# serycjon/WOFT

Hardware: AMD Instinct MI355X
Metric: tracked frames/sec at 1080p, 12 RAFT iters; flow EPE vs reference (higher is better)
Workload: dtype bf16x3 (split-bf16 MFMA operands emulating fp32, fp32 accumulate)

## Files before the change

### include/woft_hip.h

```cpp
#ifndef WOFT_HIP_H
#define WOFT_HIP_H

#include <stdint.h>

#ifdef __cplusplus
extern "C" {
#endif

#define WOFT_OK 0
#define WOFT_EINVAL (-1)
#define WOFT_ELAUNCH (-2)

int woft_abi_version(void);
int woft_sizeof(int which);
int woft_set_tuning(int key, int value);

enum woft_epilogue {
    WOFT_EPI_LINEAR = 0,
    WOFT_EPI_RELU = 1,
    WOFT_EPI_SIGMOID = 2,
    WOFT_EPI_TANH = 3,
    WOFT_EPI_RELU_RES_RELU = 4,
    WOFT_EPI_GRU_ZR = 5,
    WOFT_EPI_GRU_Q = 6,
// ... 63 lines not shown
int woft_flow_head_update(const float* in, int32_t cs, int32_t h, int32_t w, int32_t cin_pad, const float* wgt,
                          const float* bias, float* delta, int64_t ld_delta, float* coords1, float* flow4,
                          float* flow_cat, int32_t ld_cat, void* stream);
int woft_flow_head_gather(const float* part, int32_t n_planes, int32_t ld, int32_t h, int32_t w, const float* bias2,
                          float* delta, int64_t ld_delta, float* coords1, float* flow4, float* flow_cat, int32_t ld_cat,
                          void* stream);
int woft_split_bf16_lines(const float* x, int64_t n, void* out, void* stream);
int woft_corr_gemm_bf16(const void* a, const void* b, int64_t m, int64_t n, int64_t rows_a, int64_t rows_b, int32_t k,
                        float alpha, void* out, int64_t ldo, int32_t terms, int32_t out_bf16, void* stream);

int woft_inorm_finalize(const float* stat_sum, const float* stat_sq, int32_t n_part, int32_t ld,
                        int32_t channels, int32_t channels_pad, int64_t count, float eps,
                        float* mean, float* rstd, void* ws, void* stream);
int64_t woft_inorm_ws_bytes(void);
int woft_inorm_apply(const float* x, const float* mean, const float* rstd, const float* res,
                     const float* res_mean, const float* res_rstd, int32_t res_mode,
                     float* out, int64_t n_pix, int32_t channels, int32_t mode, void* stream);

int woft_preprocess_bgr_u8(const uint8_t* img, int32_t h, int32_t w, float* out,
                           int32_t hp, int32_t wp, int32_t pad_top, int32_t pad_left, void* stream);

int woft_avgpool2_nhwc(const float* in, int32_t h, int32_t w, int32_t c, float* out, void* stream);

int woft_feature_pyramid(const float* in, int32_t h, int32_t w, int32_t c, int32_t levels, float* const* pooled,
                         void* const* split, int32_t terms, void* stream);

typedef struct woft_lookup_params {
    const void* vol[4];
    int32_t ht[4], wt[4];
    int64_t plane[4];
    int32_t levels, radius;
    const float* coords;
    int64_t n_pix;
    float* out;
    int32_t ldo;
    int32_t vol_bf16;
    int32_t ablate;
} woft_lookup_params;
int woft_corr_lookup(const woft_lookup_params* p, void* stream);
typedef struct woft_lookup_otf_params {
    const void* f1;
    const void* f2[4];
    int32_t h[4], w[4];
    int32_t levels, radius, terms;
    int32_t hf, wf, k;
    float alpha;
    const float* coords;
    float* out;
    const int32_t* need;
    int32_t ldo;
    int32_t ablate;
    const float* fh_part;
    const float* fh_bias;
    float* fh_delta;
    float* fh_flow4;
    float* fh_flow_cat;
    int32_t fh_planes, fh_ld, fh_ld_delta, fh_ld_cat;
    int32_t roi_y0, roi_x0, roi_h, roi_w;
    int32_t smp_y0, smp_x0, smp_h, smp_w;
} woft_lookup_otf_params;
int woft_corr_lookup_otf(const woft_lookup_otf_params* p, void* stream);
int woft_tile_rows(const float* in, int32_t h, int32_t w, int32_t c, float* out, void* stream);

int woft_coords_update(float* coords1, const float* delta, int32_t ld_delta, int32_t wf, int64_t n_pix,
                       float* flow4, float* flow_cat, int32_t ld_cat, void* stream);
int woft_coords_init(float* coords1, int32_t hf, int32_t wf, float* flow4, float* flow_cat,
                     int32_t ld_cat, void* stream);
int woft_coords_init_flow(float* coords1, const float* flow_init, int32_t hf, int32_t wf, float* flow4, float* flow_cat,
                          int32_t ld_cat, void* stream);
int woft_forward_interpolate(const float* flow, int32_t hf, int32_t wf, float* out, void* stream);

int woft_colsum(const float* f, int64_t n_pix, int32_t c, double* ws, int32_t n_part, double* total, void* stream);
int woft_wh_conv0(const float* lookup, int32_t ld_lookup, const float* mean, int64_t n_pix, int32_t nwin,
                  const float* wt, const float* bias, float* out, const int32_t* index, void* stream);
int woft_wh_pack(const float* lookup, int32_t ld_lookup, const float* f1, int32_t c, const double* f2_total,
                 float alpha, int64_t n_pix, int32_t nwin, float* mean, float* x8, void* stream);
int woft_wh_reduce(const float* act, int32_t c, int32_t nwin2, const float* w, float bias,
                   int64_t n_pix, float* out, void* stream);
int woft_warp_features(const float* f, int32_t h, int32_t w, int32_t c, int32_t cs, const float* coords, int64_t n_pix,
                       float* out, int32_t ld_out, void* stream);
int woft_wh_needed(const float* pts, const int32_t* count, int32_t n_max, int32_t top, int32_t left, int32_t hf, int32_t wf,
                   const int32_t* index, int32_t n_win, int32_t* bitmap, int32_t* dyn_index, int32_t* n_needed, void* stream);

int woft_convex_upsample(const float* coords1, const float* wlow, const float* mask, int32_t ld_mask,
                         int32_t hf, int32_t wf, int32_t crop_top, int32_t crop_left, int32_t h, int32_t w,
                         float* flow_up, float* dst, float* wout, int32_t do_sigmoid, void* stream);
int woft_convex_weights_at(const float* pts, const int32_t* count, int32_t n_max, const float* wlow, const float* mask,
                           int32_t ld_mask, int32_t hf, int32_t wf, int32_t crop_top, int32_t crop_left,
                           int32_t do_sigmoid, float* wsel, void* stream);
int woft_flow_to_tc(const float* flow, const float* weights, int32_t h, int32_t w, float* dst, float* wout,
                    int32_t do_sigmoid, void* stream);
int woft_upflow8(const float* coords1, const float* wlow, int32_t hf, int32_t wf,
                 int32_t crop_top, int32_t crop_left, int32_t h, int32_t w,
                 float* flow_up, float* dst, float* wout, int32_t do_sigmoid, void* stream);

int woft_warp_perspective_u8(const uint8_t* img, int32_t h, int32_t w, int32_t c, const double* hinv,
                             uint8_t* out, uint8_t* valid, int32_t nearest, void* stream);

int woft_warp_perspective_window_u8(const uint8_t* img, int32_t h, int32_t w, int32_t c, const double* hinv, int32_t y0,
                                    int32_t x0, int32_t hw, int32_t ww, uint8_t* out, uint8_t* valid, int32_t nearest,
                                    void* stream);
int woft_crop_u8(const uint8_t* img, int32_t h, int32_t w, int32_t c, int32_t y0, int32_t x0, int32_t hw, int32_t ww,
                 uint8_t* out, void* stream);
int64_t woft_mask_bbox_ws_bytes(void);
int woft_mask_bbox(const uint8_t* mask, int32_t h, int32_t w, const double* hinv, uint8_t* warped, void* ws, int32_t* bbox,
                   void* stream);

int woft_resize_linear_u8(const uint8_t* img, int32_t h, int32_t w, int32_t c, uint8_t* out, int32_t ho, int32_t wo,
                          float scale_y, float scale_x, void* stream);

int64_t woft_tc_select_ws_bytes(int64_t n);
int woft_tc_select(const float* dst, const float* w, const uint8_t* tmask, const uint8_t* pwmask, int32_t gh,
                   int32_t gw, int32_t mh, int32_t mw, int32_t check_dst, const float* sobol_u, int32_t n_draw,
                   void* ws, float* pa, float* pb, float* wout, int32_t cap, int32_t* count, void* stream);
int woft_tc_flags(const float* dst, const uint8_t* tmask, const uint8_t* pwmask, int32_t gh, int32_t gw, int32_t mh,
                  int32_t mw, int32_t check_dst, uint8_t* flags, void* stream);
int woft_tc_select_vis(const float* dst, const float* w, const uint8_t* tmask, const uint8_t* pwmask, int32_t gh,
                       int32_t gw, int32_t mh, int32_t mw, int32_t check_dst, const float* sobol_u, int32_t n_draw,
                       const float* vis, int32_t vis_mode, float vis_thr, void* ws, float* pa, float* pb, float* wout,
                       int32_t cap, int32_t* count, void* stream);
int woft_tc_flags_vis(const float* dst, const uint8_t* tmask, const uint8_t* pwmask, int32_t gh, int32_t gw, int32_t mh,
                      int32_t mw, int32_t check_dst, const float* vis, int32_t vis_mode, float vis_thr, uint8_t* flags,
                      void* stream);

#define WOFT_HFIT_SINGLE_MAX 2048
int64_t woft_hfit_ws_bytes(void);
int woft_hfit(const float* pa, const float* pb, const float* w, int32_t n_max, const int32_t* count,
              int32_t reweight, float huber_k, int32_t n_irls, void* ws, float* Hout, int32_t* status, void* stream);
#define WOFT_HFIT_BATCH_MAX 65535
int woft_hfit_batched(const float* pa, const float* pb, const float* w, int32_t batch, int32_t n_max,
                      const int32_t* counts, int32_t reweight, float huber_k, int32_t n_irls, float* Hout,
                      int32_t* status, void* stream);
int woft_hfit_batched_bwd(const float* pa, const float* pb, const float* w, int32_t batch, int32_t n_max,
                          const int32_t* counts, const float* gH, float* gpa, float* gpb, float* gw, int32_t* status,
                          void* stream);
int woft_hfit_step(const float* pa, const float* pb, const float* w, int32_t n, const float* rew, int32_t first,
                   void* ws, float* res, float* Hout, int32_t* status, void* stream);
int woft_inlier_frac(const float* pa, const float* pb, int32_t n_max, const int32_t* count, const float* H,
                     float thr, float* frac, void* stream);

int64_t woft_ransac_ws_bytes(int32_t n_max, int32_t max_iters);
int woft_ransac(const float* pa, const float* pb, int32_t n_max, const int32_t* count, int32_t max_iters, double thr,
                double conf, uint64_t seed, int32_t refine, void* ws, float* Hout, int32_t* status, int32_t* info,
                uint8_t* inlier_mask, void* stream);

int64_t woft_trs_ws_bytes(int32_t n_max, int32_t max_iters);
int woft_trs(const float* pa, const float* pb, int32_t n_max, const int32_t* count, int32_t max_iters, double thr,
             double conf, uint64_t seed, int32_t refine, void* ws, float* Hout, int32_t* status, int32_t* info,
             uint8_t* inlier_mask, void* stream);

#ifdef __cplusplus
}
#endif
#endif
```

### woft_amd/_lib.py

```python
import ctypes as C
import os
from pathlib import Path

import torch

LIB_PATH = Path(os.environ.get("WOFT_HIP_LIB") or Path(__file__).resolve().parent / "lib" / "libwoft_hip.so")

EPI_LINEAR, EPI_RELU, EPI_SIGMOID, EPI_TANH, EPI_RELU_RES_RELU, EPI_GRU_ZR, EPI_GRU_Q, EPI_CTX, EPI_WH_MEAN, EPI_FLOWHEAD = range(10)

vp, i32, i64, f32 = C.c_void_p, C.c_int32, C.c_int64, C.c_float


class ConvParams(C.Structure):
    _fields_ = [
        ("in0", vp), ("in1", vp), ("cs0", i32), ("cs1", i32), ("c_split", i32),
        ("n_img", i32), ("h", i32), ("w", i32), ("ho", i32), ("wo", i32),
        ("taps_y", i32), ("taps_x", i32), ("stride", i32), ("pad_y", i32), ("pad_x", i32),
        ("cin_pad", i32), ("flat", i32), ("wgt", vp), ("wgt_hi", vp), ("wgt_lo", vp), ("precision", i32),
        ("bias", vp), ("alpha", f32),
        ("cout", i32), ("cout_pad", i32), ("out", vp), ("ldo", i64), ("co_off", i32),
        ("out_w", i32), ("out_pitch", i32), ("epi", i32), ("split", i32),
        ("e0", vp), ("e1", vp), ("lde0", i32), ("lde1", i32), ("out1", vp), ("ldo1", i32),
        ("stat_sum", vp), ("stat_sq", vp), ("tile_m", i32), ("tile_n", i32), ("halo", i32),
        ("in_norm", i32), ("in_mean", vp), ("in_rstd", vp), ("bias_map", vp), ("ld_bias_map", i32),
        ("out_index", vp),
        ("wh0_lookup", vp), ("wh0_ld", i32), ("wh0_mean", vp), ("wh0_w", vp), ("wh0_bias", vp), ("wh0_index", vp),
        ("wgt_frag", vp), ("wgt_mx", vp),
        ("roi_y0", i32), ("roi_x0", i32), ("roi_h", i32), ("roi_w", i32),
    ]


class LookupParams(C.Structure):
    _fields_ = [
        ("vol", vp * 4), ("ht", i32 * 4), ("wt", i32 * 4), ("plane", i64 * 4),
        ("levels", i32), ("radius", i32), ("coords", vp), ("n_pix", i64), ("out", vp), ("ldo", i32),
        ("vol_bf16", i32), ("ablate", i32),
    ]


class LookupOtfParams(C.Structure):
    _fields_ = [
        ("f1", vp), ("f2", vp * 4), ("h", i32 * 4), ("w", i32 * 4),
        ("levels", i32), ("radius", i32), ("terms", i32), ("hf", i32), ("wf", i32), ("k", i32),
        ("alpha", f32), ("coords", vp), ("out", vp), ("need", vp), ("ldo", i32), ("ablate", i32),
        ("fh_part", vp), ("fh_bias", vp), ("fh_delta", vp), ("fh_flow4", vp), ("fh_flow_cat", vp),
        ("fh_planes", i32), ("fh_ld", i32), ("fh_ld_delta", i32), ("fh_ld_cat", i32),
        ("roi_y0", i32), ("roi_x0", i32), ("roi_h", i32), ("roi_w", i32),
        ("smp_y0", i32), ("smp_x0", i32), ("smp_h", i32), ("smp_w", i32),
    ]


_SIGS = {
    "woft_abi_version": (i32, []),
    "woft_sizeof": (i32, [i32]),
    "woft_set_tuning": (i32, [i32, i32]),
    "woft_conv2d": (i32, [C.POINTER(ConvParams), vp]),
    "woft_conv2d_pair": (i32, [C.POINTER(ConvParams), C.POINTER(ConvParams), vp]),
    "woft_upload_u8": (i32, [vp, vp, vp, i64, i32, vp]),
    "woft_split_bf16": (i32, [vp, i64, vp, vp, vp]),
    "woft_split_bf16_lines": (i32, [vp, i64, vp, vp]),
    "woft_flow_to_tc": (i32, [vp, vp, i32, i32, vp, vp, i32, vp]),
    "woft_corr_lookup_otf": (i32, [C.POINTER(LookupOtfParams), vp]),
    "woft_conv3x3_narrow": (i32, [vp, i32, i32, i32, i32, i32, vp, vp, i32, vp, i64, i32, vp]),
    "woft_flow_head_update": (i32, [vp, i32, i32, i32, i32, vp, vp, vp, i64, vp, vp, vp, i32, vp]),
    "woft_flow_head_gather": (i32, [vp, i32, i32, i32, i32, vp, vp, i64, vp, vp, vp, i32, vp]),
    "woft_corr_gemm_bf16": (i32, [vp, vp, i64, i64, i64, i64, i32, f32, vp, i64, i32, i32, vp]),
    "woft_inorm_finalize": (i32, [vp, vp, i32, i32, i32, i32, i64, f32, vp, vp, vp, vp]),
    "woft_inorm_ws_bytes": (i64, []),
    "woft_inorm_apply": (i32, [vp, vp, vp, vp, vp, vp, i32, vp, i64, i32, i32, vp]),
    "woft_preprocess_bgr_u8": (i32, [vp, i32, i32, vp, i32, i32, i32, i32, vp]),
    "woft_avgpool2_nhwc": (i32, [vp, i32, i32, i32, vp, vp]),
    "woft_feature_pyramid": (i32, [vp, i32, i32, i32, i32, vp, vp, i32, vp]),
    "woft_corr_lookup": (i32, [C.POINTER(LookupParams), vp]),
    "woft_tile_rows": (i32, [vp, i32, i32, i32, vp, vp]),
    "woft_coords_update": (i32, [vp, vp, i32, i32, i64, vp, vp, i32, vp]),
    "woft_coords_init": (i32, [vp, i32, i32, vp, vp, i32, vp]),
    "woft_coords_init_flow": (i32, [vp, vp, i32, i32, vp, vp, i32, vp]),
    "woft_forward_interpolate": (i32, [vp, i32, i32, vp, vp]),
    "woft_colsum": (i32, [vp, i64, i32, vp, i32, vp, vp]),
    "woft_wh_pack": (i32, [vp, i32, vp, i32, vp, f32, i64, i32, vp, vp, vp]),
    "woft_wh_conv0": (i32, [vp, i32, vp, i64, i32, vp, vp, vp, vp, vp]),
    "woft_wh_reduce": (i32, [vp, i32, i32, vp, f32, i64, vp, vp]),
    "woft_warp_features": (i32, [vp, i32, i32, i32, i32, vp, i64, vp, i32, vp]),
    "woft_wh_needed": (i32, [vp, vp, i32, i32, i32, i32, i32, vp, i32, vp, vp, vp, vp]),
    "woft_convex_upsample": (i32, [vp, vp, vp, i32, i32, i32, i32, i32, i32, i32, vp, vp, vp, i32, vp]),
    "woft_convex_weights_at": (i32, [vp, vp, i32, vp, vp, i32, i32, i32, i32, i32, i32, vp, vp]),
    "woft_upflow8": (i32, [vp, vp, i32, i32, i32, i32, i32, i32, vp, vp, vp, i32, vp]),
    "woft_warp_perspective_u8": (i32, [vp, i32, i32, i32, C.POINTER(C.c_double), vp, vp, i32, vp]),
    "woft_resize_linear_u8": (i32, [vp, i32, i32, i32, vp, i32, i32, f32, f32, vp]),
    "woft_warp_perspective_window_u8": (i32, [vp, i32, i32, i32, C.POINTER(C.c_double), i32, i32, i32, i32, vp, vp, i32, vp]),
    "woft_crop_u8": (i32, [vp, i32, i32, i32, i32, i32, i32, i32, vp, vp]),
    "woft_mask_bbox_ws_bytes": (i64, []),
    "woft_mask_bbox": (i32, [vp, i32, i32, C.POINTER(C.c_double), vp, vp, vp, vp]),
    "woft_tc_select_ws_bytes": (i64, [i64]),
    "woft_tc_select": (i32, [vp, vp, vp, vp, i32, i32, i32, i32, i32, vp, i32, vp, vp, vp, vp, i32, vp, vp]),
    "woft_tc_flags": (i32, [vp, vp, vp, i32, i32, i32, i32, i32, vp, vp]),
    "woft_tc_select_vis": (i32, [vp, vp, vp, vp, i32, i32, i32, i32, i32, vp, i32, vp, i32, f32, vp, vp, vp, vp, i32, vp, vp]),
    "woft_tc_flags_vis": (i32, [vp, vp, vp, i32, i32, i32, i32, i32, vp, i32, f32, vp, vp]),
    "woft_hfit_ws_bytes": (i64, []),
    "woft_hfit": (i32, [vp, vp, vp, i32, vp, i32, f32, i32, vp, vp, vp, vp]),
    "woft_hfit_batched": (i32, [vp, vp, vp, i32, i32, vp, i32, f32, i32, vp, vp, vp]),
    "woft_hfit_batched_bwd": (i32, [vp, vp, vp, i32, i32, vp, vp, vp, vp, vp, vp, vp]),
    "woft_hfit_step": (i32, [vp, vp, vp, i32, vp, i32, vp, vp, vp, vp, vp]),
    "woft_inlier_frac": (i32, [vp, vp, i32, vp, vp, f32, vp, vp]),
    "woft_ransac_ws_bytes": (i64, [i32, i32]),
    "woft_ransac": (i32, [vp, vp, i32, vp, i32, C.c_double, C.c_double, C.c_uint64, i32, vp, vp, vp, vp, vp, vp]),
    "woft_trs_ws_bytes": (i64, [i32, i32]),
    "woft_trs": (i32, [vp, vp, i32, vp, i32, C.c_double, C.c_double, C.c_uint64, i32, vp, vp, vp, vp, vp, vp]),
}

EXPORTS = tuple(_SIGS)
_lib = None


class WoftHipError(RuntimeError):
    pass


def load():
    global _lib
    if _lib is not None:
        return _lib
    if not LIB_PATH.exists():
        raise WoftHipError(f"{LIB_PATH} is missing: build it with `python -m woft_amd.build` "
                           "(hipcc --offload-arch=gfx950); woft_amd has no CPU fallback")
    lib = C.CDLL(str(LIB_PATH))
    for name, (res, args) in _SIGS.items():
        fn = getattr(lib, name)
        fn.restype, fn.argtypes = res, args
    if lib.woft_sizeof(0) != C.sizeof(ConvParams) or lib.woft_sizeof(1) != C.sizeof(LookupParams) \
            or lib.woft_sizeof(2) != C.sizeof(LookupOtfParams):
        raise WoftHipError("ctypes mirror of woft_conv_params / woft_lookup_params is out of sync with the library")
    _lib = lib
    return lib


def check(rc, what):
    if rc != 0:
        raise WoftHipError(f"{what} failed with code {rc}")


def ptr(t):
    return None if t is None else t.data_ptr()


_RAW_STREAM = getattr(torch._C, "_cuda_getCurrentRawStream", None) if os.environ.get("WOFT_RAW_STREAM", "1") != "0" else None
_CUR_DEV = torch.cuda.current_device


def stream_ptr():
    if _RAW_STREAM is None:
        return torch.cuda.current_stream().cuda_stream
    return _RAW_STREAM(_CUR_DEV())
```

### woft_amd/csrc/hfit.hip

```cpp
#include "common.h"
#include <algorithm>

namespace {

constexpr int HT = 1024;
constexpr int NG = 45;

__device__ __forceinline__ double wave_sum(double v) {
#pragma unroll
    for (int o = 32; o > 0; o >>= 1) v += __shfl_xor(v, o);
    return v;
}

template <int CNT>
__device__ void block_sum(double (&vals)[CNT], double* red , double* out ) {
    const int lane = threadIdx.x & 63, wave = threadIdx.x >> 6;
#pragma unroll
    for (int i = 0; i < CNT; ++i) {
        const double s = wave_sum(vals[i]);
        if (lane == 0) red[wave * CNT + i] = s;
    }
    __syncthreads();
    if ((int)threadIdx.x < CNT) {
        double s = 0.0;
        for (int wv = 0; wv < HT / 64; ++wv) s += red[wv * CNT + threadIdx.x];
        out[threadIdx.x] = s;
    }
    __syncthreads();
}

__device__ __forceinline__ void build_rows(float x1, float y1, float x2, float y2, float wv, float (&rx)[9],
                                           float (&ry)[9]) {
    rx[0] = 0.f; rx[1] = 0.f; rx[2] = 0.f; rx[3] = -x1; rx[4] = -y1; rx[5] = -1.f; rx[6] = y2 * x1; rx[7] = y2 * y1;
    rx[8] = -y2;
    ry[0] = x1; ry[1] = y1; ry[2] = 1.f; ry[3] = 0.f; ry[4] = 0.f; ry[5] = 0.f; ry[6] = -x2 * x1; ry[7] = -x2 * y1;
    ry[8] = x2;
#pragma unroll
    for (int k = 0; k < 9; ++k) {
        rx[k] *= wv;
        ry[k] *= wv;
    }
}

__device__ __forceinline__ float reweight_fn(float r, int mode, float k) {
    const float a = fabsf(r);
    if (mode == 2 && a < k) return 1.f;
    return 1.f / (a + 1e-8f);
}

__device__ __forceinline__ void hfit_one(const float* __restrict__ pa, const float* __restrict__ pb,
                                         const float* __restrict__ w, int n, int reweight, float huber_k, int n_solves,
                                         float* __restrict__ Hout, int* __restrict__ status) {
    __shared__ double red[(HT / 64) * 81];
    __shared__ double tot[NG];
    __shared__ double gram[81];
    __shared__ float sol_s[8];
    __shared__ int fail_s;
    if (n < 4) {
        if (threadIdx.x == 0) {
            status[0] = 1;
            for (int i = 0; i < 9; ++i) Hout[i] = nanf("");
        }
        return;
    }
    if (threadIdx.x == 0) fail_s = 0;

    double s4[4] = {0.0, 0.0, 0.0, 0.0};
    for (int i = threadIdx.x; i < n; i += HT) {
        s4[0] += (double)pa[2 * i];
        s4[1] += (double)pa[2 * i + 1];
        s4[2] += (double)pb[2 * i];
        s4[3] += (double)pb[2 * i + 1];
    }
    block_sum<4>(s4, red, tot);
    const float m1x = (float)(tot[0] / n), m1y = (float)(tot[1] / n);
    const float m2x = (float)(tot[2] / n), m2y = (float)(tot[3] / n);
    __syncthreads();
    double d2[2] = {0.0, 0.0};
    for (int i = threadIdx.x; i < n; i += HT) {
        const float ax = pa[2 * i] - m1x, ay = pa[2 * i + 1] - m1y;
        const float bx = pb[2 * i] - m2x, by = pb[2 * i + 1] - m2y;
        d2[0] += (double)sqrtf(ax * ax + ay * ay);
        d2[1] += (double)sqrtf(bx * bx + by * by);
    }
    block_sum<2>(d2, red, tot);
    const float s1 = sqrtf(2.0f) / ((float)(tot[0] / n) + 1e-8f);
    const float s2 = sqrtf(2.0f) / ((float)(tot[1] / n) + 1e-8f);
    const float t1x = -s1 * m1x, t1y = -s1 * m1y, t2x = -s2 * m2x, t2y = -s2 * m2y;
    __syncthreads();

    typedef double f64x4 __attribute__((ext_vector_type(4)));
    const int lane = threadIdx.x & 63, wave = threadIdx.x >> 6;
    const int ec = lane & 15, ek = lane >> 4;
    for (int it = 0; it < n_solves; ++it) {
        float sol[8];
#pragma unroll
        for (int k = 0; k < 8; ++k) sol[k] = (it > 0) ? sol_s[k] : 0.f;
        f64x4 g4 = {0.0, 0.0, 0.0, 0.0};
        for (int base = wave * 2; base < n; base += (HT / 64) * 2) {
            const int i = base + (ek >> 1);
            double val = 0.0;
            if (i < n && ec < 9) {
                const float x1 = s1 * pa[2 * i] + t1x, y1 = s1 * pa[2 * i + 1] + t1y;
                const float x2 = s2 * pb[2 * i] + t2x, y2 = s2 * pb[2 * i + 1] + t2y;
                const float wv = (w != nullptr) ? w[i] : 1.f;
                float rx[9], ry[9];
                build_rows(x1, y1, x2, y2, wv, rx, ry);
                float q = 1.f;
                if (it > 0 && reweight != 0) {
                    float resx = -rx[8], resy = -ry[8];
#pragma unroll
                    for (int k = 0; k < 8; ++k) {
                        resx += rx[k] * sol[k];
                        resy += ry[k] * sol[k];
                    }
                    q = sqrtf(reweight_fn((ek & 1) ? resy : resx, reweight, huber_k));
                }
                float e = 0.f;
#pragma unroll
                for (int k = 0; k < 9; ++k)
                    if (k == ec) e = (ek & 1) ? ry[k] : rx[k];
                val = (double)(e * q);
            }
            g4 = __builtin_amdgcn_mfma_f64_16x16x4f64(val, val, g4, 0, 0, 0);
        }
#pragma unroll
        for (int r = 0; r < 4; ++r) {
            const int row = ek + 4 * r;
            if (row < 9 && ec < 9) red[wave * 81 + row * 9 + ec] = g4[r];
        }
        __syncthreads();
        if (threadIdx.x < 81) {
            double sacc = 0.0;
            for (int wv = 0; wv < HT / 64; ++wv) sacc += red[wv * 81 + threadIdx.x];
            gram[threadIdx.x] = sacc;
        }
        __syncthreads();
        if (threadIdx.x == 0) {
            double L[8][8], rhs[8];
            double G[9][9];
            for (int a = 0; a < 9; ++a)
                for (int b = 0; b < 9; ++b) G[a][b] = gram[a * 9 + b];
            bool ok = true;
            for (int i = 0; i < 8 && ok; ++i) {
                for (int j = 0; j <= i; ++j) {
                    double s = G[i][j];
                    for (int k = 0; k < j; ++k) s -= L[i][k] * L[j][k];
                    if (i == j) {
                        if (!(s > 0.0)) { ok = false; break; }
                        L[i][i] = sqrt(s);
                    } else {
                        L[i][j] = s / L[j][j];
                    }
                }
            }
            if (ok) {
                for (int i = 0; i < 8; ++i) {
                    double s = G[i][8];
                    for (int k = 0; k < i; ++k) s -= L[i][k] * rhs[k];
                    rhs[i] = s / L[i][i];
                }
                for (int i = 7; i >= 0; --i) {
                    double s = rhs[i];
                    for (int k = i + 1; k < 8; ++k) s -= L[k][i] * rhs[k];
                    rhs[i] = s / L[i][i];
                }
                for (int i = 0; i < 8; ++i) sol_s[i] = (float)rhs[i];
            } else {
                fail_s = 1;
            }
        }
        __syncthreads();
        if (fail_s) break;
    }

    if (threadIdx.x == 0) {
        if (fail_s) {
            status[0] = 2;
            for (int i = 0; i < 9; ++i) Hout[i] = nanf("");
            return;
        }
        const double hn[9] = {sol_s[0], sol_s[1], sol_s[2], sol_s[3], sol_s[4], sol_s[5], sol_s[6], sol_s[7], 1.0};
        const double T1[9] = {s1, 0, t1x, 0, s1, t1y, 0, 0, 1};
        const double i2 = 1.0 / (double)s2;
        const double T2i[9] = {i2, 0, -(double)t2x * i2, 0, i2, -(double)t2y * i2, 0, 0, 1};
        double tmp[9], hh[9];
        for (int r = 0; r < 3; ++r)
            for (int c = 0; c < 3; ++c) {
                double s = 0;
                for (int k = 0; k < 3; ++k) s += hn[r * 3 + k] * T1[k * 3 + c];
                tmp[r * 3 + c] = s;
            }
        for (int r = 0; r < 3; ++r)
            for (int c = 0; c < 3; ++c) {
                double s = 0;
                for (int k = 0; k < 3; ++k) s += T2i[r * 3 + k] * tmp[k * 3 + c];
                hh[r * 3 + c] = s;
            }
        const double den = hh[8] + 1e-8;
        for (int i = 0; i < 9; ++i) Hout[i] = (float)(hh[i] / den);
        status[0] = 0;
    }
}

__global__ __launch_bounds__(HT) void hfit_kernel(const float* __restrict__ pa, const float* __restrict__ pb,
                                                  const float* __restrict__ w, int n_max,
                                                  const int* __restrict__ count, int reweight, float huber_k,
                                                  int n_solves, float* __restrict__ Hout, int* __restrict__ status) {
    int n = n_max;
    if (count != nullptr) n = min(count[0], n_max);
    hfit_one(pa, pb, w, n, reweight, huber_k, n_solves, Hout, status);
}

__global__ __launch_bounds__(HT) void hfit_batched_kernel(const float* __restrict__ pa, const float* __restrict__ pb,
                                                          const float* __restrict__ w, int n_max,
                                                          const int* __restrict__ counts, int reweight, float huber_k,
                                                          int n_solves, float* __restrict__ Hout,
                                                          int* __restrict__ status) {
    const int b = blockIdx.x;
    const int64_t off = (int64_t)b * n_max;
    int n = n_max;
    if (counts != nullptr) n = min(counts[b], n_max);
    hfit_one(pa + 2 * off, pb + 2 * off, (w != nullptr) ? w + off : nullptr, n, reweight, huber_k, n_solves, Hout + 9 * b,
             status + b);
}


__device__ __forceinline__ bool chol8_factor(const double* gram, double (&L)[36]) {
    bool ok = true;
#pragma unroll
    for (int i = 0; i < 8; ++i) {
#pragma unroll
        for (int j = 0; j <= i; ++j) {
            double s = gram[i * 9 + j];
#pragma unroll
            for (int k = 0; k < j; ++k) s -= L[i * (i + 1) / 2 + k] * L[j * (j + 1) / 2 + k];
            if (i == j) {
                ok = ok && (s > 0.0);
                L[i * (i + 1) / 2 + i] = sqrt(s);
            } else {
                L[i * (i + 1) / 2 + j] = s / L[j * (j + 1) / 2 + j];
            }
        }
    }
    return ok;
}

__device__ __forceinline__ void chol8_solve_f64(const double (&L)[36], double (&rhs)[8]) {
#pragma unroll
    for (int i = 0; i < 8; ++i) {
        double s = rhs[i];
#pragma unroll
        for (int k = 0; k < i; ++k) s -= L[i * (i + 1) / 2 + k] * rhs[k];
        rhs[i] = s / L[i * (i + 1) / 2 + i];
    }
#pragma unroll
    for (int i = 7; i >= 0; --i) {
        double s = rhs[i];
#pragma unroll
        for (int k = i + 1; k < 8; ++k) s -= L[k * (k + 1) / 2 + i] * rhs[k];
        rhs[i] = s / L[i * (i + 1) / 2 + i];
    }
}

__device__ __forceinline__ void bwd_zero_rows(float* __restrict__ gpa, float* __restrict__ gpb, float* __restrict__ gw, int from,
                                              int n_max) {
    for (int i = from + (int)threadIdx.x; i < n_max; i += HT) {
        if (gpa != nullptr) ((float2*)gpa)[i] = make_float2(0.f, 0.f);
        if (gpb != nullptr) ((float2*)gpb)[i] = make_float2(0.f, 0.f);
        if (gw != nullptr) gw[i] = 0.f;
    }
}

__device__ __forceinline__ void hfit_bwd_one(const float* __restrict__ pa, const float* __restrict__ pb,
                                             const float* __restrict__ w, int n, int n_max, const float* __restrict__ gout,
                                             float* __restrict__ gpa, float* __restrict__ gpb, float* __restrict__ gw,
                                             int* __restrict__ status) {
    __shared__ double red[(HT / 64) * 81];
    __shared__ double tot[NG];
    __shared__ double gram[81];
    __shared__ double bw[24];
    __shared__ int fail_s;
    if (n < 4) {
        bwd_zero_rows(gpa, gpb, gw, 0, n_max);
        if (threadIdx.x == 0 && status != nullptr) status[0] = 1;
        return;
    }

    double s4[4] = {0.0, 0.0, 0.0, 0.0};
    for (int i = threadIdx.x; i < n; i += HT) {
        s4[0] += (double)pa[2 * i];
        s4[1] += (double)pa[2 * i + 1];
        s4[2] += (double)pb[2 * i];
        s4[3] += (double)pb[2 * i + 1];
    }
    block_sum<4>(s4, red, tot);
    const float m1x = (float)(tot[0] / n), m1y = (float)(tot[1] / n);
    const float m2x = (float)(tot[2] / n), m2y = (float)(tot[3] / n);
    __syncthreads();
    double d2[2] = {0.0, 0.0};
    for (int i = threadIdx.x; i < n; i += HT) {
        const float ax = pa[2 * i] - m1x, ay = pa[2 * i + 1] - m1y;
        const float bx = pb[2 * i] - m2x, by = pb[2 * i + 1] - m2y;
        d2[0] += (double)sqrtf(ax * ax + ay * ay);
        d2[1] += (double)sqrtf(bx * bx + by * by);
    }
    block_sum<2>(d2, red, tot);
    const float den1 = (float)(tot[0] / n) + 1e-8f, den2 = (float)(tot[1] / n) + 1e-8f;
    const float s1 = sqrtf(2.0f) / den1;
    const float s2 = sqrtf(2.0f) / den2;
    const float t1x = -s1 * m1x, t1y = -s1 * m1y, t2x = -s2 * m2x, t2y = -s2 * m2y;
    __syncthreads();

    typedef double f64x4 __attribute__((ext_vector_type(4)));
    const int lane = threadIdx.x & 63, wave = threadIdx.x >> 6;
    const int ec = lane & 15, ek = lane >> 4;
    {
        f64x4 g4 = {0.0, 0.0, 0.0, 0.0};
        for (int base = wave * 2; base < n; base += (HT / 64) * 2) {
            const int i = base + (ek >> 1);
            double val = 0.0;
            if (i < n && ec < 9) {
                const float x1 = s1 * pa[2 * i] + t1x, y1 = s1 * pa[2 * i + 1] + t1y;
                const float x2 = s2 * pb[2 * i] + t2x, y2 = s2 * pb[2 * i + 1] + t2y;
                const float wv = (w != nullptr) ? w[i] : 1.f;
                float rx[9], ry[9];
                build_rows(x1, y1, x2, y2, wv, rx, ry);
                float e = 0.f;
#pragma unroll
                for (int k = 0; k < 9; ++k)
                    if (k == ec) e = (ek & 1) ? ry[k] : rx[k];
                val = (double)e;
            }
            g4 = __builtin_amdgcn_mfma_f64_16x16x4f64(val, val, g4, 0, 0, 0);
        }
#pragma unroll
        for (int r = 0; r < 4; ++r) {
            const int row = ek + 4 * r;
            if (row < 9 && ec < 9) red[wave * 81 + row * 9 + ec] = g4[r];
        }
        __syncthreads();
        if (threadIdx.x < 81) {
            double sacc = 0.0;
            for (int wv = 0; wv < HT / 64; ++wv) sacc += red[wv * 81 + threadIdx.x];
            gram[threadIdx.x] = sacc;
        }
// ... 98 lines not shown
                for (int k = 0; k < 8; ++k) {
                    aUx += (double)ax[k] * bw[8 + k];
                    aXx += (double)ax[k] * bw[k];
                    aUy += (double)ay[k] * bw[8 + k];
                    aXy += (double)ay[k] * bw[k];
                }
                gw[i] = (float)((vX * (double)ax[8] - (rX * aUx + vX * aXx)) + (vY * (double)ay[8] - (rY * aUy + vY * aXy)));
            }
            if (want_pts) {
                const double W = (double)wv, X1 = x1, Y1 = y1, X2 = x2, Y2 = y2;
                const double gAx3 = -(rX * bw[11] + vX * bw[3]), gAx4 = -(rX * bw[12] + vX * bw[4]);
                const double gAx6 = -(rX * bw[14] + vX * bw[6]), gAx7 = -(rX * bw[15] + vX * bw[7]);
                const double gAy0 = -(rY * bw[8] + vY * bw[0]), gAy1 = -(rY * bw[9] + vY * bw[1]);
                const double gAy6 = -(rY * bw[14] + vY * bw[6]), gAy7 = -(rY * bw[15] + vY * bw[7]);
                gpn[j][0] = W * (-gAx3 + Y2 * gAx6 + gAy0 - X2 * gAy6);
                gpn[j][1] = W * (-gAx4 + Y2 * gAx7 + gAy1 - X2 * gAy7);
                gpn[j][2] = W * (-X1 * gAy6 - Y1 * gAy7 + vY);
                gpn[j][3] = W * (X1 * gAx6 + Y1 * gAx7 - vX);
                cen[j][0] = (double)pax - (double)m1x;
                cen[j][1] = (double)pay - (double)m1y;
                cen[j][2] = (double)pbx - (double)m2x;
                cen[j][3] = (double)pby - (double)m2y;
                dots[0] += gpn[j][0] * cen[j][0] + gpn[j][1] * cen[j][1];
                dots[1] += gpn[j][2] * cen[j][2] + gpn[j][3] * cen[j][3];
            }
        }
    }
    bwd_zero_rows(nullptr, nullptr, gw, n, n_max);
    if (!want_pts) return;

    block_sum<2>(dots, red, tot);
    const double S1 = s1, S2 = s2;
    const double gs1 = tot[0] + bw[16] + bw[17] - bw[18] * (double)m1x - bw[19] * (double)m1y;
    const double gs2 = tot[1] + bw[20] + bw[21] - bw[22] * (double)m2x - bw[23] * (double)m2y;
    const double gdb1 = (-gs1 * S1 / (double)den1) / n, gdb2 = (-gs2 * S2 / (double)den2) / n;
    __syncthreads();
    double gd[2][4];
    double sums[4] = {0.0, 0.0, 0.0, 0.0};
#pragma unroll
    for (int j = 0; j < 2; ++j) {
        const int i = (int)threadIdx.x + j * HT;
#pragma unroll
        for (int k = 0; k < 4; ++k) gd[j][k] = 0.0;
        if (i < n) {
            const double da = sqrt(cen[j][0] * cen[j][0] + cen[j][1] * cen[j][1]);
            const double db = sqrt(cen[j][2] * cen[j][2] + cen[j][3] * cen[j][3]);
            const double ia = (da > 0.0) ? 1.0 / da : 0.0, ib = (db > 0.0) ? 1.0 / db : 0.0;
            gd[j][0] = S1 * gpn[j][0] + gdb1 * (cen[j][0] * ia);
            gd[j][1] = S1 * gpn[j][1] + gdb1 * (cen[j][1] * ia);
            gd[j][2] = S2 * gpn[j][2] + gdb2 * (cen[j][2] * ib);
            gd[j][3] = S2 * gpn[j][3] + gdb2 * (cen[j][3] * ib);
#pragma unroll
            for (int k = 0; k < 4; ++k) sums[k] += gd[j][k];
        }
    }
    block_sum<4>(sums, red, tot);
    const double o0 = (-tot[0] - S1 * bw[18]) / n, o1 = (-tot[1] - S1 * bw[19]) / n;
    const double o2 = (-tot[2] - S2 * bw[22]) / n, o3 = (-tot[3] - S2 * bw[23]) / n;
#pragma unroll
    for (int j = 0; j < 2; ++j) {
        const int i = (int)threadIdx.x + j * HT;
        if (i < n) {
            if (gpa != nullptr) ((float2*)gpa)[i] = make_float2((float)(gd[j][0] + o0), (float)(gd[j][1] + o1));
            if (gpb != nullptr) ((float2*)gpb)[i] = make_float2((float)(gd[j][2] + o2), (float)(gd[j][3] + o3));
        }
    }
    bwd_zero_rows(gpa, gpb, nullptr, n, n_max);
}

__global__ __launch_bounds__(HT) void hfit_batched_bwd_kernel(const float* __restrict__ pa, const float* __restrict__ pb,
                                                              const float* __restrict__ w, int n_max,
                                                              const int* __restrict__ counts, const float* __restrict__ gH,
                                                              float* __restrict__ gpa, float* __restrict__ gpb,
                                                              float* __restrict__ gw, int* __restrict__ status) {
    const int b = blockIdx.x;
    const int64_t off = (int64_t)b * n_max;
    int n = n_max;
    if (counts != nullptr) n = min(counts[b], n_max);
    hfit_bwd_one(pa + 2 * off, pb + 2 * off, (w != nullptr) ? w + off : nullptr, n, n_max, gH + 9 * b,
                 (gpa != nullptr) ? gpa + 2 * off : nullptr, (gpb != nullptr) ? gpb + 2 * off : nullptr,
                 (gw != nullptr) ? gw + off : nullptr, (status != nullptr) ? status + b : nullptr);
}

__global__ __launch_bounds__(HT) void inlier_frac_kernel(const float* __restrict__ pa, const float* __restrict__ pb,
                                                         int n_max, const int* __restrict__ count,
                                                         const float* __restrict__ H, float thr,
                                                         float* __restrict__ frac) {
    __shared__ double red[HT / 64];
    __shared__ double tot[1];
    int n = n_max;
    if (count != nullptr) n = min(count[0], n_max);
    float h[9];
    for (int i = 0; i < 9; ++i) h[i] = H[i];
    double c[1] = {0.0};
    for (int i = threadIdx.x; i < n; i += HT) {
        const float x = pa[2 * i], y = pa[2 * i + 1];
        const float px = h[0] * x + h[1] * y + h[2], py = h[3] * x + h[4] * y + h[5], pz = h[6] * x + h[7] * y + h[8];
        const float sc = (fabsf(pz) > 1e-8f) ? 1.f / (pz + 1e-8f) : 1.f;
        const float dx = sc * px - pb[2 * i], dy = sc * py - pb[2 * i + 1];
        c[0] += (sqrtf(dx * dx + dy * dy) <= thr) ? 1.0 : 0.0;
    }
    block_sum<1>(c, red, tot);
    if (threadIdx.x == 0) frac[0] = (n > 0) ? (float)(tot[0] / n) : 0.f;
}

constexpr int MT = 256;
constexpr int MAXG = 1024;

struct MWs {
    double* psum;
    double* pdist;
    double* pgram;
    float* sol;
    float* norm;
};
__host__ __device__ inline MWs mws_layout(void* ws) {
    MWs o;
    o.psum = (double*)ws;
    o.pdist = o.psum + MAXG * 4;
    o.pgram = o.pdist + MAXG * 2;
    o.sol = (float*)(o.pgram + MAXG * 81);
    o.norm = o.sol + 8;
    return o;
}
inline int mws_groups(int n_max) { return (int)std::min<int64_t>(MAXG, std::max<int64_t>(1, ((int64_t)n_max + 2047) / 2048)); }

template <int CNT>
__device__ void block_sum_m(double (&vals)[CNT], double* red , double* out ) {
    const int lane = threadIdx.x & 63, wave = threadIdx.x >> 6;
#pragma unroll
    for (int i = 0; i < CNT; ++i) {
        const double s = wave_sum(vals[i]);
        if (lane == 0) red[wave * CNT + i] = s;
    }
    __syncthreads();
    if ((int)threadIdx.x < CNT) {
        double s = 0.0;
        for (int wv = 0; wv < MT / 64; ++wv) s += red[wv * CNT + threadIdx.x];
        out[threadIdx.x] = s;
    }
}

__device__ __forceinline__ int fit_count(const int* count, int n_max) { return count ? min(count[0], n_max) : n_max; }

__global__ __launch_bounds__(MT) void hfit_sum_kernel(const float* __restrict__ pa, const float* __restrict__ pb, int n_max,
                                                      const int* __restrict__ count, void* ws) {
    __shared__ double red[(MT / 64) * 4];
    const MWs s = mws_layout(ws);
    const int n = fit_count(count, n_max);
    double v[4] = {0.0, 0.0, 0.0, 0.0};
    for (int64_t i = (int64_t)blockIdx.x * MT + threadIdx.x; i < n; i += (int64_t)gridDim.x * MT) {
        const float2 a = ((const float2*)pa)[i], b = ((const float2*)pb)[i];
        v[0] += (double)a.x; v[1] += (double)a.y; v[2] += (double)b.x; v[3] += (double)b.y;
    }
    block_sum_m<4>(v, red, s.psum + blockIdx.x * 4);
}

template <int CNT>
__device__ __forceinline__ void partial_total(const double* __restrict__ part, int G, double* out ) {
    __shared__ double tred[(MT / 64) * CNT];
    double acc[CNT];
#pragma unroll
    for (int c = 0; c < CNT; ++c) acc[c] = 0.0;
    for (int g = threadIdx.x; g < G; g += MT)
#pragma unroll
        for (int c = 0; c < CNT; ++c) acc[c] += part[(int64_t)g * CNT + c];
    const int lane = threadIdx.x & 63, wave = threadIdx.x >> 6;
#pragma unroll
    for (int c = 0; c < CNT; ++c) {
        const double t = wave_sum(acc[c]);
        if (lane == 0) tred[wave * CNT + c] = t;
    }
    __syncthreads();
    if ((int)threadIdx.x < CNT) {
        double t = 0.0;
        for (int wv = 0; wv < MT / 64; ++wv) t += tred[wv * CNT + threadIdx.x];
        out[threadIdx.x] = t;
    }
    __syncthreads();
}

__device__ __forceinline__ void fit_means(const MWs& s, int n, double* sh ) {
    partial_total<4>(s.psum, (int)gridDim.x, sh);
    if (threadIdx.x < 4) sh[threadIdx.x] /= n;
    __syncthreads();
}
// ... 177 lines not shown
    }
    {
        __shared__ double part[(ST / 64) * 81];
        const int lane = threadIdx.x & 63, wave = threadIdx.x >> 6;
        double t0 = 0.0, t1 = 0.0;
#pragma unroll 4
        for (int g = wave; g < groups; g += ST / 64) {
            t0 += s.pgram[(int64_t)g * 81 + lane];
            if (lane < 17) t1 += s.pgram[(int64_t)g * 81 + 64 + lane];
        }
        part[wave * 81 + lane] = t0;
        if (lane < 17) part[wave * 81 + 64 + lane] = t1;
        __syncthreads();
        if (threadIdx.x < 81) {
            double t = 0.0;
            for (int wv = 0; wv < ST / 64; ++wv) t += part[wv * 81 + threadIdx.x];
            gram[threadIdx.x] = t;
        }
        __syncthreads();
    }
    if (threadIdx.x == 0) {
        if (status[0] == 2) return;
        float sol[8];
        if (!cholesky_solve8(gram, sol)) {
            status[0] = 2;
            for (int i = 0; i < 9; ++i) Hout[i] = nanf("");
            for (int i = 0; i < 8; ++i) s.sol[i] = nanf("");
            return;
        }
        for (int i = 0; i < 8; ++i) s.sol[i] = sol[i];
        denormalise(sol, s.norm[0], s.norm[1], s.norm[2], s.norm[3], s.norm[4], s.norm[5], Hout);
        status[0] = 0;
    }
}

__global__ __launch_bounds__(MT) void hfit_resid_kernel(const float* __restrict__ pa, const float* __restrict__ pb,
                                                        const float* __restrict__ w, int n_max,
                                                        const int* __restrict__ count, const void* ws,
                                                        float* __restrict__ res) {
    const MWs s = mws_layout(const_cast<void*>(ws));
    const int n = fit_count(count, n_max);
    const int64_t i = (int64_t)blockIdx.x * MT + threadIdx.x;
    if (i >= n) return;
    const float s1 = s.norm[0], t1x = s.norm[1], t1y = s.norm[2], s2 = s.norm[3], t2x = s.norm[4], t2y = s.norm[5];
    const float2 a = ((const float2*)pa)[i], b = ((const float2*)pb)[i];
    float rx[9], ry[9];
    build_rows(s1 * a.x + t1x, s1 * a.y + t1y, s2 * b.x + t2x, s2 * b.y + t2y, (w != nullptr) ? w[i] : 1.f, rx, ry);
    float resx = -rx[8], resy = -ry[8];
#pragma unroll
    for (int k = 0; k < 8; ++k) {
        resx += rx[k] * s.sol[k];
        resy += ry[k] * s.sol[k];
    }
    ((float2*)res)[i] = make_float2(resx, resy);
}

}

extern "C" int64_t woft_hfit_ws_bytes(void) { return (int64_t)MAXG * (4 + 2 + 81) * 8 + 16 * 4; }

extern "C" int woft_hfit(const float* pa, const float* pb, const float* w, int32_t n_max, const int32_t* count,
                         int32_t reweight, float huber_k, int32_t n_irls, void* ws, float* Hout, int32_t* status,
                         void* stream) {
    if (!pa || !pb || !Hout || !status || n_max < 0 || reweight < 0 || reweight > 2 || n_irls < 0) return WOFT_EINVAL;
    hipStream_t st = (hipStream_t)stream;
    if (ws == nullptr || n_max <= WOFT_HFIT_SINGLE_MAX) {
        hipLaunchKernelGGL(hfit_kernel, dim3(1), dim3(HT), 0, st, pa, pb, w, n_max, count, reweight, huber_k, n_irls + 1,
                           Hout, status);
        return woft_launch_status();
    }
    const int G = mws_groups(n_max);
    (void)hipMemsetAsync(status, 0, sizeof(int32_t), st);
    hipLaunchKernelGGL(hfit_sum_kernel, dim3(G), dim3(MT), 0, st, pa, pb, n_max, count, ws);
    hipLaunchKernelGGL(hfit_dist_kernel, dim3(G), dim3(MT), 0, st, pa, pb, n_max, count, ws);
    const int solves = (reweight != 0) ? n_irls + 1 : 1;
    for (int it = 0; it < solves; ++it) {
        hipLaunchKernelGGL(hfit_gram_kernel, dim3(G), dim3(MT), 0, st, pa, pb, w, n_max, count, (const float*)nullptr,
                           reweight, huber_k, it > 0 ? 1 : 0, ws);
        hipLaunchKernelGGL(hfit_solve_kernel, dim3(1), dim3(ST), 0, st, n_max, count, G, ws, Hout, status);
    }
    return woft_launch_status();
}

extern "C" int woft_hfit_batched(const float* pa, const float* pb, const float* w, int32_t batch, int32_t n_max,
                                 const int32_t* counts, int32_t reweight, float huber_k, int32_t n_irls, float* Hout,
                                 int32_t* status, void* stream) {
    if (!pa || !pb || !Hout || !status || batch < 1 || batch > WOFT_HFIT_BATCH_MAX || n_max < 1 ||
        n_max > WOFT_HFIT_SINGLE_MAX || reweight < 0 || reweight > 2 || n_irls < 0)
        return WOFT_EINVAL;
    hipLaunchKernelGGL(hfit_batched_kernel, dim3(batch), dim3(HT), 0, (hipStream_t)stream, pa, pb, w, n_max, counts, reweight,
                       huber_k, n_irls + 1, Hout, status);
    return woft_launch_status();
}

extern "C" int woft_hfit_batched_bwd(const float* pa, const float* pb, const float* w, int32_t batch, int32_t n_max,
                                     const int32_t* counts, const float* gH, float* gpa, float* gpb, float* gw,
                                     int32_t* status, void* stream) {
    if (!pa || !pb || !gH || (!gpa && !gpb && !gw) || (gw && !w) || batch < 1 || batch > WOFT_HFIT_BATCH_MAX || n_max < 1 ||
        n_max > WOFT_HFIT_SINGLE_MAX)
        return WOFT_EINVAL;
    static_assert(WOFT_HFIT_SINGLE_MAX <= 2 * HT, "hfit_bwd_one keeps two correspondences per thread");
    hipLaunchKernelGGL(hfit_batched_bwd_kernel, dim3(batch), dim3(HT), 0, (hipStream_t)stream, pa, pb, w, n_max, counts, gH, gpa,
                       gpb, gw, status);
    return woft_launch_status();
}

extern "C" int woft_hfit_step(const float* pa, const float* pb, const float* w, int32_t n, const float* rew, int32_t first,
                              void* ws, float* res, float* Hout, int32_t* status, void* stream) {
    if (!pa || !pb || !ws || !Hout || !status || n < 0) return WOFT_EINVAL;
    hipStream_t st = (hipStream_t)stream;
    const int G = mws_groups(n);
    if (first) {
        (void)hipMemsetAsync(status, 0, sizeof(int32_t), st);
        hipLaunchKernelGGL(hfit_sum_kernel, dim3(G), dim3(MT), 0, st, pa, pb, n, (const int*)nullptr, ws);
        hipLaunchKernelGGL(hfit_dist_kernel, dim3(G), dim3(MT), 0, st, pa, pb, n, (const int*)nullptr, ws);
    }
    hipLaunchKernelGGL(hfit_gram_kernel, dim3(G), dim3(MT), 0, st, pa, pb, w, n, (const int*)nullptr, rew, 0, 0.f, 0, ws);
    hipLaunchKernelGGL(hfit_solve_kernel, dim3(1), dim3(ST), 0, st, n, (const int*)nullptr, G, ws, Hout, status);
    if (res != nullptr && n >= 4)
        hipLaunchKernelGGL(hfit_resid_kernel, dim3((n + MT - 1) / MT), dim3(MT), 0, st, pa, pb, w, n, (const int*)nullptr,
                           (const void*)ws, res);
    return woft_launch_status();
}

extern "C" int woft_inlier_frac(const float* pa, const float* pb, int32_t n_max, const int32_t* count, const float* H,
                                float thr, float* frac, void* stream) {
    if (!pa || !pb || !H || !frac || n_max < 0) return WOFT_EINVAL;
    hipLaunchKernelGGL(inlier_frac_kernel, dim3(1), dim3(HT), 0, (hipStream_t)stream, pa, pb, n_max, count, H, thr,
                       frac);
    return woft_launch_status();
}
```

### woft_amd/csrc/upsample.hip

```cpp
#include "common.h"
#include "warp_pixel.h"

namespace {

__global__ __launch_bounds__(256) void convex_upsample_kernel(
    const float* __restrict__ coords1, const float* __restrict__ wlow, const float* __restrict__ mask, int ld_mask,
    int hf, int wf, int crop_top, int crop_left, int h, int w, float* __restrict__ flow_up, float* __restrict__ dst,
    float* __restrict__ wout, int do_sigmoid) {
    const int lane = threadIdx.x & 63;
    const int64_t pix = (int64_t)blockIdx.x * 4 + (threadIdx.x >> 6);
    if (pix >= (int64_t)hf * wf) return;
    const int hc = (int)(pix / wf), wc = (int)(pix - (int64_t)hc * wf);
    const float* m = mask + pix * ld_mask + lane;
    float e[9];
    float mx = -INFINITY;
#pragma unroll
    for (int k = 0; k < 9; ++k) {
        e[k] = m[k * 64];
        mx = fmaxf(mx, e[k]);
    }
    float den = 0.f;
#pragma unroll
    for (int k = 0; k < 9; ++k) {
        e[k] = expf(e[k] - mx);
        den += e[k];
    }
    float ax = 0.f, ay = 0.f, aw = 0.f;
#pragma unroll
    for (int k = 0; k < 9; ++k) {
        const int ny = hc + k / 3 - 1, nx = wc + k % 3 - 1;
        float vx = 0.f, vy = 0.f, vw = 0.f;
        if (ny >= 0 && ny < hf && nx >= 0 && nx < wf) {
            const int64_t q = (int64_t)ny * wf + nx;
            vx = 8.f * (coords1[q * 2] - (float)nx);
            vy = 8.f * (coords1[q * 2 + 1] - (float)ny);
            if (wlow != nullptr) vw = 8.f * wlow[q];
        }
        const float s = e[k] / den;
        ax += s * vx;
        ay += s * vy;
        aw += s * vw;
    }
    const int y = 8 * hc + (lane >> 3) - crop_top, x = 8 * wc + (lane & 7) - crop_left;
    if (y < 0 || y >= h || x < 0 || x >= w) return;
    const int64_t o = (int64_t)y * w + x, hw = (int64_t)h * w;
    if (flow_up != nullptr) {
        flow_up[o] = ax;
        flow_up[hw + o] = ay;
    }
    if (dst != nullptr) {
        dst[o] = (float)x + ax;
        dst[hw + o] = (float)y + ay;
    }
    if (wout != nullptr && wlow != nullptr) {
        float v = aw / 8.f;
        if (do_sigmoid) v = sigmoidf_(v);
        wout[o] = v;
    }
}

__global__ void convex_weights_at_kernel(const float* __restrict__ pts, const int* __restrict__ count, int n_max,
                                         const float* __restrict__ wlow, const float* __restrict__ mask, int ld_mask, int hf,
                                         int wf, int crop_top, int crop_left, int do_sigmoid, float* __restrict__ wsel) {
    const int i = blockIdx.x * blockDim.x + threadIdx.x;
    const int n = count ? min(count[0], n_max) : n_max;
    if (i >= n) return;
    const int X = (int)pts[2 * i] + crop_left, Y = (int)pts[2 * i + 1] + crop_top;
    const int hc = Y >> 3, wc = X >> 3, lane = (Y & 7) * 8 + (X & 7);
    const float* m = mask + ((int64_t)hc * wf + wc) * ld_mask + lane;
    float e[9];
    float mx = -INFINITY;
#pragma unroll
    for (int k = 0; k < 9; ++k) {
        e[k] = m[k * 64];
        mx = fmaxf(mx, e[k]);
    }
    float den = 0.f;
#pragma unroll
    for (int k = 0; k < 9; ++k) {
        e[k] = expf(e[k] - mx);
        den += e[k];
    }
    float aw = 0.f;
#pragma unroll
    for (int k = 0; k < 9; ++k) {
        const int ny = hc + k / 3 - 1, nx = wc + k % 3 - 1;
        float vw = 0.f;
        if (ny >= 0 && ny < hf && nx >= 0 && nx < wf) vw = 8.f * wlow[(int64_t)ny * wf + nx];
        const float s = e[k] / den;
        aw += s * vw;
    }
    float v = aw / 8.f;
    if (do_sigmoid) v = sigmoidf_(v);
    wsel[i] = v;
}

__global__ void upflow8_kernel(const float* __restrict__ coords1, const float* __restrict__ wlow, int hf, int wf,
                               int crop_top, int crop_left, int h, int w, float* __restrict__ flow_up,
                               float* __restrict__ dst, float* __restrict__ wout, int do_sigmoid) {
    const int64_t o = (int64_t)blockIdx.x * blockDim.x + threadIdx.x;
    if (o >= (int64_t)h * w) return;
    const int y = (int)(o / w), x = (int)(o - (int64_t)y * w);
    const int Y = y + crop_top, X = x + crop_left;
    const int H8 = 8 * hf, W8 = 8 * wf;
    const float ry = (H8 > 1) ? (float)(hf - 1) / (float)(H8 - 1) : 0.f;
    const float rx = (W8 > 1) ? (float)(wf - 1) / (float)(W8 - 1) : 0.f;
    const float sy = ry * (float)Y, sx = rx * (float)X;
    const int y0 = (int)sy, x0 = (int)sx;
    const int yp = (y0 < hf - 1) ? 1 : 0, xp = (x0 < wf - 1) ? 1 : 0;
    const float ly = sy - (float)y0, lx = sx - (float)x0;
    const float hy = 1.f - ly, hx = 1.f - lx;
    const int64_t q00 = (int64_t)y0 * wf + x0, q01 = q00 + xp, q10 = q00 + (int64_t)yp * wf, q11 = q10 + xp;
    auto fl = [&](int64_t q, int ch) { return coords1[q * 2 + ch] - (float)(ch == 0 ? (q % wf) : (q / wf)); };
    const float fx = hy * (hx * fl(q00, 0) + lx * fl(q01, 0)) + ly * (hx * fl(q10, 0) + lx * fl(q11, 0));
    const float fy = hy * (hx * fl(q00, 1) + lx * fl(q01, 1)) + ly * (hx * fl(q10, 1) + lx * fl(q11, 1));
    const int64_t hw = (int64_t)h * w;
    if (flow_up != nullptr) {
        flow_up[o] = 8.f * fx;
        flow_up[hw + o] = 8.f * fy;
    }
    if (dst != nullptr) {
        dst[o] = (float)x + 8.f * fx;
        dst[hw + o] = (float)y + 8.f * fy;
    }
    if (wout != nullptr && wlow != nullptr) {
        float v = hy * (hx * wlow[q00] + lx * wlow[q01]) + ly * (hx * wlow[q10] + lx * wlow[q11]);
        v = (8.f * v) / 8.f;
        if (do_sigmoid) v = sigmoidf_(v);
        wout[o] = v;
    }
}

__global__ void warp_kernel(const uint8_t* __restrict__ img, int h, int w, int c, H9 hi, uint8_t* __restrict__ out,
                            uint8_t* __restrict__ valid, int nearest) {
    const int64_t o = (int64_t)blockIdx.x * blockDim.x + threadIdx.x;
    if (o >= (int64_t)h * w) return;
    const int y = (int)(o / w), x = (int)(o - (int64_t)y * w);
    warp_pixel(img, h, w, c, hi, x, y, o, out, valid, nearest);
}

__global__ void resize_linear_kernel(const uint8_t* __restrict__ img, int h, int w, int c, uint8_t* __restrict__ out,
                                     int ho, int wo, float sy, float sx) {
    const int64_t o = (int64_t)blockIdx.x * blockDim.x + threadIdx.x;
    if (o >= (int64_t)ho * wo) return;
    const int y = (int)(o / wo), x = (int)(o - (int64_t)y * wo);
    float fy = ((float)y + 0.5f) * sy - 0.5f, fx = ((float)x + 0.5f) * sx - 0.5f;
    int y0 = (int)floorf(fy), x0 = (int)floorf(fx);
    fy -= (float)y0;
    fx -= (float)x0;
    if (y0 < 0) { y0 = 0; fy = 0.f; }
    if (x0 < 0) { x0 = 0; fx = 0.f; }
    if (y0 >= h - 1) { y0 = h - 1; fy = 0.f; }
    if (x0 >= w - 1) { x0 = w - 1; fx = 0.f; }
    const int y1 = min(y0 + 1, h - 1), x1 = min(x0 + 1, w - 1);
    for (int k = 0; k < c; ++k) {
        const float t00 = img[((int64_t)y0 * w + x0) * c + k], t01 = img[((int64_t)y0 * w + x1) * c + k];
        const float t10 = img[((int64_t)y1 * w + x0) * c + k], t11 = img[((int64_t)y1 * w + x1) * c + k];
        const float top = t00 * (1.f - fx) + t01 * fx, bot = t10 * (1.f - fx) + t11 * fx;
        out[o * c + k] = (uint8_t)fminf(fmaxf(rintf(top * (1.f - fy) + bot * fy), 0.f), 255.f);
    }
}


__global__ void flow_to_tc_kernel(const float* __restrict__ flow, const float* __restrict__ wts, int h, int w,
                                  float* __restrict__ dst, float* __restrict__ wout, int do_sigmoid) {
    const int64_t i = (int64_t)blockIdx.x * blockDim.x + threadIdx.x;
    const int64_t n = (int64_t)h * w;
    if (i >= n) return;
    if (dst != nullptr) {
        dst[i] = (float)(i % w) + flow[i];
        dst[n + i] = (float)(i / w) + flow[n + i];
    }
    if (wts != nullptr && wout != nullptr) wout[i] = do_sigmoid ? sigmoidf_(wts[i]) : wts[i];
}

}

// ... 61 lines not shown
```

### woft_amd/csrc/wh.hip

```cpp
#include "common.h"

namespace {

__global__ void colsum_stage1(const float* __restrict__ f, int64_t n_pix, int c, double* __restrict__ partial,
                              int n_part) {
    const int64_t per = (n_pix + n_part - 1) / n_part;
    const int64_t beg = (int64_t)blockIdx.x * per;
    const int64_t end = beg + per < n_pix ? beg + per : n_pix;
    for (int ch = threadIdx.x; ch < c; ch += blockDim.x) {
        double s[8] = {0.0, 0.0, 0.0, 0.0, 0.0, 0.0, 0.0, 0.0};
        int64_t q = beg;
        for (; q + 8 <= end; q += 8) {
#pragma unroll
            for (int k = 0; k < 8; ++k) s[k] += (double)f[(q + k) * c + ch];
        }
        for (; q < end; ++q) s[0] += (double)f[q * c + ch];
        partial[(int64_t)blockIdx.x * c + ch] = ((s[0] + s[1]) + (s[2] + s[3])) + ((s[4] + s[5]) + (s[6] + s[7]));
    }
}
__global__ void colsum_stage2(const double* __restrict__ partial, int n_part, int c, double* __restrict__ total) {
    const int ch = blockIdx.x * blockDim.x + threadIdx.x;
    if (ch >= c) return;
    double s[8] = {0.0, 0.0, 0.0, 0.0, 0.0, 0.0, 0.0, 0.0};
    int b = 0;
// ... 49 lines not shown
    if (lane == 0) out[p] = bias + s / (float)nwin2;
}

template <int NW>
__global__ __launch_bounds__(256) void wh_conv0_kernel(const float* __restrict__ lookup, int ld,
                                                       const float* __restrict__ mean, int n_pix,
                                                       const float* __restrict__ wt, const float* __restrict__ b0,
                                                       float* __restrict__ out, const int* __restrict__ index) {
    typedef float f32x2 __attribute__((ext_vector_type(2)));
    const int lane = threadIdx.x & 63;
    const int wave = __builtin_amdgcn_readfirstlane(threadIdx.x >> 6);
    const int co = 2 * lane;
    f32x2 w[3][3][5];
#pragma unroll
    for (int ky = 0; ky < 3; ++ky)
#pragma unroll
        for (int kx = 0; kx < 3; ++kx)
#pragma unroll
            for (int ci = 0; ci < 5; ++ci) w[ky][kx][ci] = *(const f32x2*)(wt + (ky * 32 + kx * 8 + ci) * 128 + co);
    const f32x2 bias = *(const f32x2*)(b0 + co);
    for (int p = blockIdx.x * 4 + wave; p < n_pix; p += gridDim.x * 4) {
        const int src = index ? index[p] : p;
        if (src < 0) continue;
        const float* __restrict__ lk = lookup + (int64_t)src * ld;
        const float mv = mean[src];
        float* __restrict__ o = out + (int64_t)p * (NW * NW * 128) + co;
#pragma unroll 1
        for (int y = 0; y < NW; ++y) {
#pragma unroll
            for (int x = 0; x < NW; ++x) {
                f32x2 acc = bias;
#pragma unroll
                for (int ky = 0; ky < 3; ++ky) {
                    const int yy = y + ky - 1;
                    if (yy < 0 || yy >= NW) continue;
#pragma unroll
                    for (int kx = 0; kx < 3; ++kx) {
                        const int xx = x + kx - 1;
                        if (xx < 0 || xx >= NW) continue;
                        const float* xv = lk + (yy * NW + xx) * 4;
#pragma unroll
                        for (int ci = 0; ci < 4; ++ci) {
                            const f32x2 xs = {xv[ci], xv[ci]};
                            acc = __builtin_elementwise_fma(w[ky][kx][ci], xs, acc);
                        }
                        const f32x2 ms = {mv, mv};
                        acc = __builtin_elementwise_fma(w[ky][kx][4], ms, acc);
                    }
                }
                const f32x2 r = {fmaxf(acc[0], 0.f), fmaxf(acc[1], 0.f)};
                *(f32x2*)(o + (y * NW + x) * 128) = r;
            }
        }
    }
}

}

__global__ void wh_mark_kernel(const float* __restrict__ pts, const int* __restrict__ count, int n_max, int top, int left,
                               int hf, int wf, int* __restrict__ bitmap) {
    const int i = blockIdx.x * blockDim.x + threadIdx.x;
    const int n = count ? min(count[0], n_max) : n_max;
    if (i >= n) return;
    const int cx = ((int)pts[2 * i] + left) >> 3, cy = ((int)pts[2 * i + 1] + top) >> 3;
#pragma unroll
    for (int dy = -1; dy <= 1; ++dy)
#pragma unroll
        for (int dx = -1; dx <= 1; ++dx) {
            const int yy = cy + dy, xx = cx + dx;
            if (yy >= 0 && yy < hf && xx >= 0 && xx < wf) bitmap[yy * wf + xx] = 1;
        }
}

__global__ void wh_dyn_index_kernel(const int* __restrict__ index, int n_win, const int* __restrict__ bitmap,
                                    int* __restrict__ dyn, int* __restrict__ n_needed) {
    const int j = blockIdx.x * blockDim.x + threadIdx.x;
    if (j >= n_win) return;
    const int src = index[j];
    const bool need = bitmap[src] != 0;
    dyn[j] = need ? src : -1;
    if (need && n_needed != nullptr) atomicAdd(n_needed, 1);
}

extern "C" int woft_wh_needed(const float* pts, const int32_t* count, int32_t n_max, int32_t top, int32_t left, int32_t hf,
                              int32_t wf, const int32_t* index, int32_t n_win, int32_t* bitmap, int32_t* dyn_index,
                              int32_t* n_needed, void* stream) {
    if (!pts || !index || !bitmap || !dyn_index || n_max <= 0 || n_win <= 0 || hf <= 0 || wf <= 0) return WOFT_EINVAL;
    hipStream_t s = (hipStream_t)stream;
    (void)hipMemsetAsync(bitmap, 0, (size_t)hf * wf * sizeof(int32_t), s);
    if (n_needed) (void)hipMemsetAsync(n_needed, 0, sizeof(int32_t), s);
    hipLaunchKernelGGL(wh_mark_kernel, dim3((n_max + 255) / 256), dim3(256), 0, s, pts, count, n_max, top, left, hf, wf,
                       bitmap);
    hipLaunchKernelGGL(wh_dyn_index_kernel, dim3((n_win + 255) / 256), dim3(256), 0, s, index, n_win, bitmap, dyn_index,
                       n_needed);
    return woft_launch_status();
}

extern "C" int woft_wh_conv0(const float* lookup, int32_t ld_lookup, const float* mean, int64_t n_pix, int32_t nwin,
                             const float* wt, const float* bias, float* out, const int32_t* index, void* stream) {
    if (!lookup || !mean || !wt || !bias || !out || n_pix <= 0 || n_pix >= (1ll << 31)) return WOFT_EINVAL;
    if (ld_lookup < nwin * nwin * 4 || (nwin != 9 && nwin != 7)) return WOFT_EINVAL;
    const int64_t quads = (n_pix + 3) / 4;
    dim3 grid((unsigned)(quads < 256 * 8 ? quads : 256 * 8));
    hipStream_t s = (hipStream_t)stream;
    if (nwin == 9)
        hipLaunchKernelGGL(wh_conv0_kernel<9>, grid, dim3(256), 0, s, lookup, ld_lookup, mean, (int)n_pix, wt, bias, out, index);
    else
        hipLaunchKernelGGL(wh_conv0_kernel<7>, grid, dim3(256), 0, s, lookup, ld_lookup, mean, (int)n_pix, wt, bias, out, index);
    return woft_launch_status();
}

extern "C" int woft_colsum(const float* f, int64_t n_pix, int32_t c, double* ws, int32_t n_part, double* total,
                           void* stream) {
    if (!f || !ws || !total || n_pix <= 0 || c <= 0 || n_part <= 0) return WOFT_EINVAL;
    hipStream_t s = (hipStream_t)stream;
    hipLaunchKernelGGL(colsum_stage1, dim3(n_part), dim3(256), 0, s, f, n_pix, c, ws, n_part);
    hipLaunchKernelGGL(colsum_stage2, dim3((c + 255) / 256), dim3(256), 0, s, ws, n_part, c, total);
    return woft_launch_status();
}

extern "C" int woft_wh_pack(const float* lookup, int32_t ld_lookup, const float* f1, int32_t c, const double* f2_total,
                            float alpha, int64_t n_pix, int32_t nwin, float* mean, float* x8, void* stream) {
    if (!lookup || !f1 || !f2_total || !mean || n_pix <= 0 || nwin <= 0 || c <= 0) return WOFT_EINVAL;
    if (ld_lookup < nwin * nwin * 4 || ld_lookup % 4 != 0) return WOFT_EINVAL;
    hipStream_t s = (hipStream_t)stream;
    hipLaunchKernelGGL(wh_mean_kernel, dim3((unsigned)ceil_div64(n_pix, 4)), dim3(256), 0, s, f1, c, f2_total, alpha,
                       n_pix, mean);
    if (x8 == nullptr) return woft_launch_status();
    const int64_t n = n_pix * nwin * nwin;
    hipLaunchKernelGGL(wh_pack_kernel, dim3((unsigned)ceil_div64(n, 256)), dim3(256), 0, s, lookup, ld_lookup, mean,
                       n_pix, nwin * nwin, x8);
    return woft_launch_status();
}

extern "C" int woft_wh_reduce(const float* act, int32_t c, int32_t nwin2, const float* w, float bias, int64_t n_pix,
                              float* out, void* stream) {
    if (!act || !w || !out || c <= 0 || c % 4 != 0 || nwin2 <= 0 || n_pix <= 0) return WOFT_EINVAL;
    hipLaunchKernelGGL(wh_reduce_kernel, dim3((unsigned)ceil_div64(n_pix, 4)), dim3(256), 0, (hipStream_t)stream, act,
                       c, nwin2, w, bias, n_pix, out);
    return woft_launch_status();
}
```

### woft_amd/engine.py

```python
import math
import os

import torch

from . import _lib, flow_region, ops
from .ops import Act, new_act

EPI = _lib
DEFER_NORM = os.environ.get("WOFT_DEFER_NORM", "1") != "0"
FUSE_FLOWHEAD = os.environ.get("WOFT_FUSE_FLOWHEAD", "1") != "0"
PAIR_BRANCHES = os.environ.get("WOFT_PAIR", "1") != "0"
PYRAMID_ONE_LAUNCH = os.environ.get("WOFT_PYRAMID", "1") != "0"
FOLD_GATHER = os.environ.get("WOFT_FOLD_GATHER", "1") != "0"
ROI_HALOS = (8, 12, 16)


def _ru(x, m):
    return (x + m - 1) // m * m


class _Spec:

    def __init__(self, small):
        self.small = small
# ... 183 lines not shown
        self.f1rows = z(_ru(P, 128), sp.fdim)
        self.f1 = Act(self.f1rows[:P], 1, hf, wf, sp.fdim)
        self.prec_corr, self.prec_wh = eng.prec_corr, eng.prec_wh
        x3 = self.prec_corr == "bf16x3"
        bf = lambda rows: (torch.zeros(rows.shape[0], rows.shape[1] * (2 if x3 else 1), dtype=torch.bfloat16, device=dev)
                           if self.prec != "fp32" else None)
        self.f1s = bf(self.f1rows)
        if eng.corr == "otf" and self.prec == "fp32":
            self.f1s = self.f1rows
        self.otf = eng.corr == "otf"
        self.dims, self.f2rows, self.f2act, self.vol = [], [], [], []
        self.f2s = []
        h, w = hf, wf
        for _ in range(sp.levels):
            self.dims.append((h, w))
            self.f2act.append(new_act(1, h, w, sp.fdim, zero=True))
            if self.otf:
                self.f2s.append(bf(self.f2act[-1].t) if self.prec != "fp32" else self.f2act[-1].t)
            else:
                n = ops.tiled_dims(h, w)[2]
                rows = z(_ru(n, 128), sp.fdim)
                self.f2rows.append(rows)
                self.f2s.append(bf(rows))
                vdt = torch.bfloat16 if eng.volume_storage == "bf16" else torch.float32
                self.vol.append(torch.zeros(P, n, dtype=vdt, device=dev))
            h, w = h // 2, w // 2
        self.net0 = new_act(1, hf, wf, sp.hdim, zero=True)
        self.xbuf = new_act(1, hf, wf, sp.xdim, zero=True)
        self._enc_scratch = {}
        n_stat = 2 * math.ceil((hp // 2) * (wp // 2) / 64) * 128
        self.stats = (z(n_stat), z(n_stat))
        self.fin_ws = ops.inorm_ws(dev)
        self._norm_slots = {}
        self.prog_f_src = self._encoder_program(eng.fnet, self.img[0], [(eng.fnet.conv2, self.f1, 0, EPI.EPI_LINEAR)])
        self.prog_f_dst = self._encoder_program(eng.fnet, self.img[1],
                                                [(eng.fnet.conv2, self.f2act[0], 0, EPI.EPI_LINEAR)])
        self.prog_c_src = self._encoder_program(eng.cnet, self.img[0],
                                                [(eng.cnet.conv2_net, self.net0, 0, EPI.EPI_TANH),
                                                 (eng.cnet.conv2_inp, self.xbuf, 0, EPI.EPI_RELU)])
        self.prog_volume = self._volume_program()

        self.coords = z(P, 2)
        self.corr = new_act(1, hf, wf, sp.corr_c, cs=sp.corr_cs, zero=True)
        self.c1 = new_act(1, hf, wf, 96 if sp.small else 256, zero=True)
        self.cf = new_act(1, hf, wf, 128 if sp.small else 256, zero=True)
        self.fl1 = new_act(1, hf, wf, 64 if sp.small else 128, zero=True)
        self.flow4 = new_act(1, hf, wf, 2, cs=4, zero=True)
        self.inp_c = new_act(1, hf, wf, sp.cdim, zero=True)
        self.gate_bias = [(new_act(1, hf, wf, 2 * sp.hdim, zero=True), new_act(1, hf, wf, sp.hdim, zero=True))
                          for _ in eng.zr_inp]
        self.prog_gate_bias = []
        for k in range(len(eng.zr_inp)):
            self.prog_gate_bias += [("conv", cp(self.inp_c, eng.zr_inp[k], self.gate_bias[k][0])),
                                    ("conv", cp(self.inp_c, eng.q_inp[k], self.gate_bias[k][1]))]
        self.zbuf = new_act(1, hf, wf, sp.hdim, zero=True)
        self.rh = new_act(1, hf, wf, sp.hdim, zero=True)
        self.hA = new_act(1, hf, wf, sp.hdim, zero=True)
        self.hB = new_act(1, hf, wf, sp.hdim, zero=True)
        self.fh = new_act(1, hf, wf, 128 if sp.small else 256, zero=True)
        self.fh_part = None
        self.delta = new_act(1, hf, wf, 2, cs=4, zero=True)
        self.flow_init = z(2, hf, wf)
        if self.otf:
            self.lookup = ops.make_lookup_otf_params(self.f1s, self.f2s, self.dims, hf, wf, sp.fdim, self.coords,
                                                     self.corr.t, sp.radius, 3 if x3 else (0 if self.prec == "fp32" else 1))
        else:
            self.lookup = ops.make_lookup_params(self.vol, self.dims, self.coords, self.corr.t, sp.radius)
        self.prog_iter_first = self._iter_program(first=True)
        self.prog_iter = self._iter_program(first=False)
        self.prog_mask = []
        if not sp.small:
            self.mk = new_act(1, hf, wf, 256, zero=True)
            self.mask = new_act(1, hf, wf, 576, zero=True)
            self.prog_mask = [cp(self.hB, eng.mk1, self.mk, epi=EPI.EPI_RELU),
                              cp(self.mk, eng.mk2, self.mask)]
            self.prog_iter_last = None
            k = next((i for i, ent in enumerate(self.prog_iter) if len(ent) > 2 and ent[2] == "fh1"), None)
            if PAIR_BRANCHES and k is not None and ops.pair_ok(self.prog_iter[k][1], self.prog_mask[0]):
                self.prog_iter_last = (self.prog_iter[:k] + [("conv2", (self.prog_iter[k][1], self.prog_mask[0]), "fh1+mk1")]
                                       + self.prog_iter[k + 1:])
        self._fold = self._fold_gather_programs()
        self.flow_region = None
        self._flow_regions = {}
        if eng.weighted:
            n = sp.nwin
            self.x8 = new_act(P, n, n, 5, cs=8, zero=True)
            self.wmean = z(P)
            self.wlow = z(P)
            self.cs_ws = torch.zeros(256, sp.fdim, dtype=torch.float64, device=dev)
            self.cs_tot = torch.zeros(sp.fdim, dtype=torch.float64, device=dev)
            self.wh6_b = torch.tensor([eng.wh6_b], dtype=torch.float32, device=dev)
            self.wh_region = None
            self._wh_regions = {}
            self._wh_dyn = {}
            if eng.wh_std:
                self.a2 = new_act(P, n, n, 128)
                self.wh0_direct = n in (7, 9)
                self.wh0_fused = (eng.wh0_frag is not None and os.environ.get("WOFT_WH0_FUSED", "1") != "0"
                                  and cp(self.a2, eng.wh2, self.a2, epi=EPI.EPI_RELU, precision=self.prec_wh).halo == 2)
                self.a1 = self.a2 if self.wh0_fused else new_act(P, n, n, 128)
                self.wh0_t = eng.wh0.wgt[:128].t().contiguous()
                self.prog_wh, self.wh_fused = self._wh_program(P, None)
            else:
                self.wh0_direct = self.wh0_fused = self.wh_fused = False
                cpw = lambda *a, **kw: self._cp(*a, precision=self.prec_wh, **kw)
                x = self.x8
                if not eng.wh_flat0:
                    self.x32 = new_act(P, n, n, 5, cs=32, zero=True)
                    x = self.x32
                self.prog_wh = []
                for pc in eng.wh_layers:
                    out = new_act(P, n, n, pc.cout, cs=_ru(_ru(pc.cout, 4), 32), zero=True)
                    self.prog_wh.append(cpw(x, pc, out, epi=EPI.EPI_RELU))
                    x = out
                self.wh_last = x
        if eng.mask_head:
            self.mh_warped = new_act(1, hf, wf, sp.fdim, zero=True)
            self.prog_mh = []
            x = None
            for k, pc in enumerate(eng.mh_layers):
                out = new_act(1, hf, wf, pc.cout, cs=_ru(_ru(pc.cout, 4), 32), zero=True)
                if k == 0:
                    self.prog_mh.append(self._cp(self.f1, pc, out, x2=self.mh_warped, c_split=sp.fdim, epi=EPI.EPI_RELU,
                                                 precision=self.prec_wh))
                else:
                    self.prog_mh.append(self._cp(x, pc, out, epi=EPI.EPI_RELU, precision=self.prec_wh))
                x = out
            self.mh_last = x
            self.mh_w = torch.zeros(x.cs, dtype=torch.float32)
            self.mh_w[:eng.mh_c] = eng.mh_wlast
            self.mh_w = self.mh_w.to(dev)
            self.mh_low = z(P)

    def _fold_gather_programs(self):
        progs = [self.prog_iter_first, self.prog_iter] + ([self.prog_iter_last] if getattr(self, "prog_iter_last", None) else [])
        if not (FOLD_GATHER and self.otf and all(p and p[-1][0] == "fh_gather" and p[0][0] == "lookup" for p in progs)):
            return None
        n_planes, bias2 = self.prog_iter[-1][1]
        lk = type(self.lookup).from_buffer_copy(self.lookup)
        off = self.eng.spec.flow_off
        flow_cat = self.xbuf.t[:, off:]
        lk.fh_part, lk.fh_bias, lk.fh_delta = _lib.ptr(self.fh_part), _lib.ptr(bias2), _lib.ptr(self.delta.t)
        lk.fh_flow4, lk.fh_flow_cat = _lib.ptr(self.flow4.t), flow_cat.data_ptr()
        lk.fh_planes, lk.fh_ld, lk.fh_ld_delta, lk.fh_ld_cat = n_planes, self.fh_part.shape[1], self.delta.cs, self.xbuf.cs
        lk._keep = (self.lookup._keep, bias2, self.fh_part)
        out = {"gather": [self.prog_iter[-1]], "lookup": lk}
        for p in progs:
            head = p[0] if p is self.prog_iter_first else ("lookup", lk)
            out[id(p)] = [head] + p[1:-1]
        return out

    def _wh_program(self, n_win, index):
        eng, n = self.eng, self.eng.spec.nwin
        cp = lambda *a, **kw: self._cp(*a, precision=self.prec_wh, **kw)
        a1 = Act(self.a1.t[:n_win * n * n], n_win, n, n, 128)
        a2 = Act(self.a2.t[:n_win * n * n], n_win, n, n, 128)
        prog = ([] if self.wh0_direct else [cp(self.x8, eng.wh0, a1, epi=EPI.EPI_RELU)]) + [
            cp(a1, eng.wh2, a2, epi=EPI.EPI_RELU), cp(a2, eng.wh4, a1, epi=EPI.EPI_RELU)]
        if self.wh0_fused:
            assert prog[0].halo == 2
            prog[0] = cp(a1, eng.wh2, a2, epi=EPI.EPI_RELU,
                         wh0=(self.corr, self.wmean, eng.wh0_frag, eng.wh0.bias, index))
        last = prog[-1]
        fused = last.halo == 2
        if fused:
            last.epi = EPI.EPI_WH_MEAN
# ... 248 lines not shown
        return prog

    def run(self, prog):
        for ent in prog:
            kind, a = ent[0], ent[1]
            if kind == "conv2":
                ev = self.conv_events
                if ev is not None and len(ent) > 2 and ent[2] in ev:
                    s, t = torch.cuda.Event(enable_timing=True), torch.cuda.Event(enable_timing=True)
                    s.record()
                    ops.run_conv_pair(*a)
                    t.record()
                    ev[ent[2]].append((s, t))
                else:
                    ops.run_conv_pair(*a)
            elif kind == "conv":
                ev = self.conv_events
                if ev is not None and len(ent) > 2 and ent[2] in ev:
                    s, t = torch.cuda.Event(enable_timing=True), torch.cuda.Event(enable_timing=True)
                    s.record()
                    ops.run_conv(a)
                    t.record()
                    ev[ent[2]].append((s, t))
                else:
                    ops.run_conv(a)
            elif kind == "fin":
                rows, ld, c, c_pad, count, ms = a
                ops.inorm_finalize(self.stats, rows, ld, c, count, ms[0], ms[1], channels_pad=c_pad, ws=self.fin_ws)
            elif kind == "apply":
                raw, out, mode, res, ms, res_ms, res_mode = a
                ops.inorm_apply(raw, ms[0], ms[1], out, mode, res=res, res_stats=res_ms, res_mode=res_mode)
            elif kind == "pyramid":
                ops.feature_pyramid(a)
            elif kind == "pool":
                ops.avgpool2(a[0], a[1])
            elif kind == "split":
                self._split(a[0], a[1])
            elif kind == "tile":
                ops.tile_rows(a[0], a[1])
            elif kind == "cgemm":
                ops.corr_gemm_bf16(*a)
            elif kind == "narrow":
                ops.conv3x3_narrow(*a)
            elif kind == "lookup":
                self._lookup(a)
            elif kind == "copy":
                a[1].copy_(a[0])
            elif kind == "fh_gather":
                off = self.eng.spec.flow_off
                ops.flow_head_gather(self.fh_part, a[0], self.hf, self.wf, a[1], self.delta, self.coords, self.flow4.t,
                                     self.xbuf.t[:, off:], self.xbuf.cs)
            elif kind == "fh_update":
                off = self.eng.spec.flow_off
                ops.flow_head_update(a[0], a[1], a[2], self.coords, self.flow4.t, self.xbuf.t[:, off:], self.xbuf.cs)
            elif kind == "coords":
                off = self.eng.spec.flow_off
                ops.coords_update(self.coords, self.delta.t, self.delta.cs, self.wf, self.flow4.t,
                                  self.xbuf.t[:, off:], self.xbuf.cs)
            else:
                raise ValueError(kind)

    def _lookup(self, params):
        run = ops.run_lookup_otf if self.otf else ops.run_lookup
        if self.lookup_events is None:
            run(params)
            return
        s, e = torch.cuda.Event(enable_timing=True), torch.cuda.Event(enable_timing=True)
        s.record()
        run(params)
        e.record()
        self.lookup_events.append((s, e))

    def _split(self, rows, out):
        if self.prec_corr == "bf16x3":
            ops.split_bf16_lines(rows, out)
        else:
            ops.split_bf16(rows, out, None)

    def load_image(self, slot, img_u8, pad_top, pad_left):
        ops.preprocess(img_u8, self.img[slot], self.hp, self.wp, pad_top, pad_left)

    def encode_source(self, reuse_target=False):
        reused = bool(reuse_target) and self.otf and getattr(self, "target_valid", False)
        if reused:
            self.f1rows[:self.P].copy_(self.f2act[0].t.view(self.P, -1))
            if self.prec != "fp32":
                self.f1s[:self.P].copy_(self.f2s[0])
        else:
            self.run(self.prog_f_src)
        self.run(self.prog_c_src)
        if self.prec != "fp32" and not reused:
            self._split(self.f1rows, self.f1s)
        if self.gate_bias is not None:
            self.inp_c.t.copy_(self.xbuf.t[:, :self.eng.spec.cdim])
            self.run(self.prog_gate_bias)
        return reused

    def set_flow_init(self, flow_init):
        if tuple(flow_init.shape) != (2, self.hf, self.wf):
            raise ValueError(f"flow_init must have shape (2, {self.hf}, {self.wf}) for a {self.hp} x {self.wp} padded input, "
                             f"got {tuple(flow_init.shape)}")
        self.flow_init.copy_(flow_init, non_blocking=True)

    def flow_low(self):
        return self.flow4.t[:, :2].t().reshape(2, self.hf, self.wf).contiguous()

    def flow(self, iters, crop, h, w, flow_up=None, dst=None, wout=None, do_sigmoid=False, trace=None, defer_wh=False,
             mout=None, mask_sigmoid=False, flow_init=None):
        e, sp = self.eng, self.eng.spec
        if iters < 1:
            raise ValueError("iters must be >= 1")
        self.run(self.prog_f_dst)
        self.run(self.prog_volume)
        self.target_valid = True
        off = sp.flow_off
        if flow_init is None:
            ops.coords_init(self.coords, self.hf, self.wf, self.flow4.t, self.xbuf.t[:, off:], self.xbuf.cs)
        else:
            if flow_init is not True:
                self.set_flow_init(flow_init)
            ops.coords_init_flow(self.coords, self.flow_init, self.hf, self.wf, self.flow4.t, self.xbuf.t[:, off:], self.xbuf.cs)
            if trace is not None:
                trace(self, -1)
        last = getattr(self, "prog_iter_last", None) if iters > 1 else None
        fold = self._fold if trace is None else None
        region = self.flow_region if (trace is None and flow_init is None) else None
        if region is not None and region["key"][1] != iters:
            region = None
        for it in range(iters):
            prog = self.prog_iter_first if it == 0 else (last if (last is not None and it == iters - 1) else self.prog_iter)
            if fold is not None:
                prog = fold[id(prog)]
            if region is not None:
                prog = region["iters"].get(it, prog)
            self.run(prog)
            if trace is not None:
                trace(self, it)
        if fold is not None:
            self.run(fold["gather"])
        for p in (self.prog_mask[1:] if last is not None else self.prog_mask):
            ops.run_conv(p)
        wlow = None
        if defer_wh:
            assert e.weighted and not sp.small and self.wh_region is not None and not e.mask_head
            ops.convex_upsample(self.coords, None, self.mask.t, self.hf, self.wf, crop, h, w, flow_up=flow_up, dst=dst,
                                wout=None, do_sigmoid=do_sigmoid)
            return
        if e.weighted:
            self._weight_head(self.wh_region[1] if self.wh_region is not None else self.prog_wh,
                              self.wh_region[0] if self.wh_region is not None else None)
            wlow = self.wlow
        wout = wout if e.weighted else None
        if sp.small:
            ops.upflow8(self.coords, wlow, self.hf, self.wf, crop, h, w, flow_up=flow_up, dst=dst, wout=wout,
                        do_sigmoid=do_sigmoid)
        else:
            ops.convex_upsample(self.coords, wlow, self.mask.t, self.hf, self.wf, crop, h, w, flow_up=flow_up,
                                dst=dst, wout=wout, do_sigmoid=do_sigmoid)
        if e.mask_head:
            self._mask_head()
            if mout is not None:
                if sp.small:
                    ops.upflow8(self.coords, self.mh_low, self.hf, self.wf, crop, h, w, wout=mout, do_sigmoid=mask_sigmoid)
                else:
                    ops.convex_upsample(self.coords, self.mh_low, self.mask.t, self.hf, self.wf, crop, h, w, wout=mout,
                                        do_sigmoid=mask_sigmoid)

    def _mask_head(self):
        e = self.eng
        ops.warp_features(self.f2act[0], self.coords, self.mh_warped)
        for p in self.prog_mh:
            ops.run_conv(p)
        last = self.mh_last
        _lib.check(_lib.load().woft_wh_reduce(_lib.ptr(last.t), last.cs, 1, _lib.ptr(self.mh_w), e.mh_b, self.P,
                                              _lib.ptr(self.mh_low), _lib.stream_ptr()), "woft_wh_reduce")

    def finish_weights(self, pts, count, n_max, pad, crop, h, w, flow_up=None, dst=None, wout=None, do_sigmoid=False,
                       w_points=None):
        index, _ = self.wh_region[:2]
        key = index.data_ptr()
        if key not in self._wh_dyn:
            dyn = torch.full_like(index, -1)
            prog, fused = self._wh_program(int(index.numel()), dyn)
            assert fused
            self._wh_dyn[key] = (dyn, prog, torch.zeros(self.P, dtype=torch.int32, device=index.device),
                                 torch.zeros(1, dtype=torch.int32, device=index.device))
        dyn, prog, bitmap, n_needed = self._wh_dyn[key]
        ops.wh_needed(pts, count, n_max, pad[0], pad[1], self.hf, self.wf, index, bitmap, dyn, n_needed)
        self._weight_head(prog, dyn, n_needed, need=bitmap)
        if w_points is not None:
            ops.convex_weights_at(pts, count, n_max, self.wlow, self.mask.t, self.hf, self.wf, crop, w_points,
                                  do_sigmoid=do_sigmoid)
            return
        ops.convex_upsample(self.coords, self.wlow, self.mask.t, self.hf, self.wf, crop, h, w, flow_up=flow_up, dst=dst,
                            wout=wout, do_sigmoid=do_sigmoid)

    def _wh6_padded(self, cs):
        if getattr(self, "_wh6_pad", None) is None or self._wh6_pad.numel() != cs:
            self._wh6_pad = torch.zeros(cs, dtype=torch.float32, device="cuda")
            self._wh6_pad[:self.eng.wh6_c] = self.eng.wh6_w[:self.eng.wh6_c]
        return self._wh6_pad

    def _weight_head(self, prog_wh, index, n_needed=None, need=None):
        e, sp = self.eng, self.eng.spec
        if need is not None and self.otf:
            self.lookup.need = _lib.ptr(need)
            self._lookup(self.lookup)
            self.lookup.need = None
        else:
            self._lookup(self.lookup)
        lib = _lib.load()
        n = sp.nwin
        _lib.check(lib.woft_colsum(_lib.ptr(self.f2act[0].t), self.P, sp.fdim, _lib.ptr(self.cs_ws), 256,
                                   _lib.ptr(self.cs_tot), _lib.stream_ptr()), "woft_colsum")
        _lib.check(lib.woft_wh_pack(_lib.ptr(self.corr.t), self.corr.cs, _lib.ptr(self.f1.t), sp.fdim,
                                    _lib.ptr(self.cs_tot), 1.0 / (math.sqrt(float(sp.fdim)) * self.P), self.P, n,
                                    _lib.ptr(self.wmean), None if self.wh0_direct else _lib.ptr(self.x8.t),
                                    _lib.stream_ptr()), "woft_wh_pack")
        if not e.wh_std and not e.wh_flat0:
            self.x32.t[:, :8].copy_(self.x8.t)
        n_win = int(index.numel()) if index is not None else self.P
        if index is not None:
            self.wlow.zero_()
        if self.wh0_direct and not self.wh0_fused:
            _lib.check(lib.woft_wh_conv0(_lib.ptr(self.corr.t), self.corr.cs, _lib.ptr(self.wmean), n_win, n,
                                         _lib.ptr(self.wh0_t), _lib.ptr(e.wh0.bias), _lib.ptr(self.a1.t),
                                         _lib.ptr(index) if index is not None else None,
                                         _lib.stream_ptr()), "woft_wh_conv0")
        for k, p in enumerate(prog_wh):
            if k == 0 and self.wh_events is not None:
                s, t = torch.cuda.Event(enable_timing=True), torch.cuda.Event(enable_timing=True)
                s.record()
                ops.run_conv(p)
                t.record()
                self.wh_events.append((s, t, n_win if n_needed is None else n_needed.clone()))
            else:
                ops.run_conv(p)
        if not self.wh_fused:
            last = self.a1 if e.wh_std else self.wh_last
            _lib.check(lib.woft_wh_reduce(_lib.ptr(last.t), last.cs, n * n, _lib.ptr(self._wh6_padded(last.cs)), e.wh6_b, self.P,
                                          _lib.ptr(self.wlow), _lib.stream_ptr()), "woft_wh_reduce")
```

### woft_amd/flow_provider.py

```python
import logging
import os
from collections import OrderedDict
from pathlib import Path
from timeit import default_timer as timer

import numpy as np
import torch

from . import _lib, ops
from .engine import RaftEngine

logger = logging.getLogger(__name__)


def _pad_geometry(h, w, mode):
    if mode == "nopad":
        assert h % 8 == 0
        assert w % 8 == 0
        return h, w, 0, 0, h, w, h, w
    if mode == "crop":
        ch, cw = (h // 8) * 8, (w // 8) * 8
        return ch, cw, 0, 0, ch, cw, ch, cw
    if mode == "RAFT":
        ph = (((h // 8) + 1) * 8 - h) % 8
# ... 12 lines not shown
        for c, k in layers:
            c, k = int(c), int(k)
            if c < 1 or k < 1 or k % 2 == 0:
                raise ValueError
            shapes.append((c, cur, k, k))
            cur = c
    except (TypeError, ValueError):
        raise ValueError(f"class_params.mask_head_structure {structure!r}: not a list of (channels, odd kernel) tuples "
                         "or channel counts (weighted_raft.py:387-409)") from None
    return shapes + [(1, cur, 1, 1)]


class _Recent:

    def __init__(self):
        self.order, self.protected = OrderedDict(), None

    def touch(self, key, keep, protect=False):
        if protect:
            self.protected = key
        self.order[key] = None
        self.order.move_to_end(key)
        others = [k for k in self.order if k != self.protected]
        dropped = others[:max(0, len(others) - keep)]
        for k in dropped:
            del self.order[k]
        return dropped


class RAFTWrapper:
    def __init__(self, config):
        self.C = config
        cp = config.class_params
        if self.C.raft_type not in ("orig", "weighted", "weighted_masked"):
            raise ValueError(f"Unknown RAFT type {self.C.raft_type}")
        self.masked = self.C.raft_type == "weighted_masked"
        if self.masked and not cp.mask_estimation:
            raise ValueError("raft_type 'weighted_masked' needs class_params.mask_estimation = True (and mask_head_structure): "
                             "without the MaskHead the network has no mask output")
        if self.C.raft_type == "weighted" and cp.mask_estimation:
            raise ValueError("class_params.mask_estimation is set with raft_type 'weighted', which returns no mask: use raft_type "
                             "'weighted_masked'")
        self._cache_mask_warned = False
        logger.info(f"Loading weights from: {self.C.model}")

        def read(src):
            sd = src if isinstance(src, dict) else torch.load(src, map_location="cpu")
            return {(k[len("module."):] if k.startswith("module.") else k): v for k, v in sd.items()}
        state_dict = read(self.C.model)
        if self.C.backbone_model:
            in_backbone = lambda k: ("fnet" in k) or ("cnet" in k) or ("update_block" in k)
            state_dict = {k: v for k, v in state_dict.items() if not in_backbone(k)}
            state_dict.update({k: v for k, v in read(self.C.backbone_model).items() if in_backbone(k)})
        weighted = self.C.raft_type in ("weighted", "weighted_masked")
        small = bool(cp.small)
        if self.masked:
            if not cp.mask_head_structure:
                raise ValueError("raft_type 'weighted_masked' needs class_params.mask_head_structure (weighted_raft.py:387-409)")
            want = _mask_head_shapes(cp.mask_head_structure, 128 if small else 256)
            idx = sorted(int(k.split(".")[2]) for k in state_dict if k.startswith("mask_head.net.") and k.endswith(".weight"))
            got = [tuple(state_dict[f"mask_head.net.{i}.weight"].shape) for i in idx]
            if got != want or idx != list(range(0, 2 * len(want), 2)):
                raise ValueError(f"class_params.mask_head_structure {cp.mask_head_structure!r} expects mask_head.net layers {want}; "
                                 f"the checkpoint has {got} (at net.{idx})")
        for src, val in (("env WOFT_PRECISION", os.environ.get("WOFT_PRECISION")),
                         ("flow config key 'precision'", self.C.precision),
                         ("class_params.mixed_precision", "fp16" if cp.mixed_precision else None),
                         ("built-in default (no key in the flow config): fp32-emulating bf16x3 -- finer than the TF32 convolutions "
                          "the reference's torch 1.8.1 runs by default on Ampere; 'fp32' = exact products", "bf16x3")):
            if val:
                self.precision, self.precision_source = str(val), src
                break
        note = (f"RAFT arithmetic: precision = '{self.precision}' (from: {self.precision_source}). "
                + ("This is the reference's arithmetic (exact IEEE fp32 products)." if self.precision == "fp32" else
                   "NOT the reference's IEEE-fp32 products: set precision = 'fp32' in the flow config (or WOFT_PRECISION=fp32) "
                   "for the reference's arithmetic (about 4x slower)."))
        logger.log(logging.WARNING if self.precision_source.startswith("built-in default") else logging.INFO, note)
        self.precision_note = note
        self.corr = os.environ.get("WOFT_CORR") or getattr(self.C, "corr", None) or "otf"
        self.engine = RaftEngine(state_dict, small=small, weighted=weighted, precision=self.precision, corr=self.corr,
                                 volume_storage=getattr(self.C, "volume_storage", None), mask_head=self.masked)
        v = getattr(self.C, "flow_region", None)
        self.flow_region_on = (os.environ.get("WOFT_FLOW_REGION", "1") != "0") if (v is None or isinstance(v, type(self.C))) else bool(v)
        self.use_graph = (os.environ.get("WOFT_GRAPH") or str(int(bool(getattr(self.C, "graph", False))))) == "1"
        self._pinned = None
        self._pinned_key = None
        self._wmask, self._wregion, self._all_pixels = None, {}, {}
        self._fmask, self._fregion = None, {}
        self.weights_deferred, self._deferred = False, None
        self.defer_min_ratio = 6
        self._out = {}
        self._cache_errors = set()
        self._last_dst = {}
        self.source_features_reused = False
        self._plan_bound = None
        self._recent_plans, self._recent_outs, self._recent_pixels = _Recent(), _Recent(), _Recent()

    def bound_plans(self, n_other):
        self._plan_bound = None if n_other is None else max(1, int(n_other))

    def _touch_plan(self, plan_key, out_key, n_pix, pinned_here):
        n = self._plan_bound
        if n is None:
            return
        for key in self._recent_plans.touch(plan_key, n, protect=pinned_here):
            plan = self.engine.drop_plan(key)
            self._last_dst.pop(id(plan), None)
        for key in self._recent_outs.touch(out_key, n, protect=pinned_here):
            self._out.pop(key, None)
        for key in self._recent_pixels.touch(n_pix, n, protect=pinned_here):
            self._all_pixels.pop(key, None)

    def _run_flow(self, plan, iters, crop, oh, ow, o, weighted, do_sigmoid, defer_wh=False, want_flow=True, mask_sigmoid=False,
                  has_init=False):
        def eager():
            plan.flow(iters, crop, oh, ow, flow_up=o["flow"] if want_flow else None, dst=o["dst"], wout=o["w"] if weighted else None,
                      do_sigmoid=do_sigmoid, defer_wh=defer_wh, mout=o.get("m"), mask_sigmoid=mask_sigmoid,
                      flow_init=True if has_init else None)
        if not self.use_graph or plan.lookup_events is not None or plan.wh_events is not None or plan.conv_events is not None:
            return eager()
        graphs = plan.__dict__.setdefault("_graphs", {})
        region = plan.wh_region
        fregion = plan.flow_region if not has_init else None
        key = (iters, crop, oh, ow, weighted, do_sigmoid, want_flow, bool(defer_wh), o["flow"].data_ptr(),
               region[0].data_ptr() if region is not None else 0, bool(mask_sigmoid), bool(has_init),
               fregion["key"] if fregion is not None else None)
        g = graphs.get(key)
        if g is None:
            eager()
            if key in graphs:
                g = torch.cuda.CUDAGraph()
                with torch.cuda.graph(g):
                    eager()
            graphs[key] = g
        else:
            g.replay()

    def finish_weights(self, pts, count, n_max, out=None):
        plan, crop, oh, ow, o, do_sigmoid = self._deferred
        self._deferred = None
        plan.finish_weights(pts, count, n_max, crop, crop, oh, ow, flow_up=o["flow"], dst=o["dst"], wout=o["w"],
                            do_sigmoid=do_sigmoid, w_points=out)
        return o["w"] if out is None else out

    def pin_source(self, src_img):
        self._pinned = src_img
        self._pinned_key = None
        self._wmask, self._wregion = None, {}
        self._fmask, self._fregion = None, {}

    def pin_flow_region(self, mask):
        self._fmask = None if mask is None else np.ascontiguousarray(np.asarray(mask) > 0)
        self._fregion = {}

    def _flow_region(self, key, hp, wp, top, left, oh, ow):
        if self._fmask is None:
            return None
        if key not in self._fregion:
            ys, xs = np.nonzero(self._fmask[:oh, :ow])
            rect = None
            if ys.size:
                y0, y1, x0, x1 = (ys.min() + top) >> 3, (ys.max() + top) >> 3, (xs.min() + left) >> 3, (xs.max() + left) >> 3
                rect = (int(y0), int(x0), int(y1 - y0 + 1), int(x1 - x0 + 1))
            self._fregion[key] = rect
        return self._fregion[key]

    def pin_weight_region(self, mask):
        self._wmask = None if mask is None else np.ascontiguousarray(np.asarray(mask) > 0)
        self._wregion = {}

    def _weight_region(self, key, hp, wp, top, left, oh, ow):
        if self._wmask is None:
            return None
        if key not in self._wregion:
            m = self._wmask[:oh, :ow]
            coarse = np.zeros((hp // 8, wp // 8), bool)
            ys, xs = np.nonzero(m)
            coarse[(ys + top) >> 3, (xs + left) >> 3] = True
            pad = np.pad(coarse, 1)
            dil = np.zeros_like(coarse)
            for dy in range(3):
                for dx in range(3):
                    dil |= pad[dy:dy + coarse.shape[0], dx:dx + coarse.shape[1]]
            idx = np.flatnonzero(dil).astype(np.int32)
            self._wregion[key] = torch.from_numpy(idx).cuda() if idx.size and idx.size < dil.size else None
        return self._wregion[key]

    def postprocess_weights(self, flat_weights, fn):
        s = self.last_flow_shape
        weights = fn(flat_weights.reshape(s["batch"], 1, s["H"], s["W"]))
        return weights.reshape(s["batch"], s["H"] * s["W"])

    def _outputs(self, h, w):
        key = (h, w)
        if key not in self._out:
            z = lambda *s: torch.empty(*s, dtype=torch.float32, device="cuda")
            self._out[key] = dict(flow=z(2, h, w), dst=z(2, h * w), w=z(1, h * w),
                                  src=torch.stack([torch.arange(h * w, device="cuda") % w,
                                                   torch.div(torch.arange(h * w, device="cuda"), w, rounding_mode="floor")]))
            if self.masked:
                self._out[key]["m"] = z(1, h * w)
        return self._out[key]

    def _cached_flow(self, src_img, identifier, mode, numpy_out, do_sigmoid, borrow=False):
        dataset_name, seq_name, frame_i = identifier
        path = Path(self.C.flow_cache_dir) / dataset_name / seq_name / f"{frame_i}-{frame_i + 1}.npz"
        data = np.load(path, allow_pickle=False)
        flow = np.ascontiguousarray(data["half_flow"].astype(np.float32))
        wts = data["half_weights"].astype(np.float32)
        wts = np.ascontiguousarray(wts) if wts.size > 1 else None
        h, w = flow.shape[1:]
        post = self.C.weights_postprocessing_fn if wts is not None else None
        o = self._outputs(h, w)
        o["flow"].copy_(torch.from_numpy(flow), non_blocking=True)
        wl = None
        if wts is not None:
            wl = torch.from_numpy(wts).cuda(non_blocking=True)
        lib = _lib.load()
        _lib.check(lib.woft_flow_to_tc(_lib.ptr(o["flow"]), _lib.ptr(wl), h, w, _lib.ptr(o["dst"]),
                                       _lib.ptr(o["w"]) if wl is not None else None, int(bool(do_sigmoid) and not post),
                                       _lib.stream_ptr()), "woft_flow_to_tc")
        if post:
            self._postprocess_logits(o, h, w, do_sigmoid)
# ... 31 lines not shown
            raise ValueError(f"flow_init must be a float array of shape {want} or {(1,) + want} (1/8-resolution pixels of the "
                             f"{hp} x {wp} padded image), got {tuple(flow_init.shape)} {flow_init.dtype}")
        return t.detach().to(torch.float32)

    def flow_key(self, src_img):
        hp, wp, top, left = _pad_geometry(src_img.shape[0], src_img.shape[1], self.C.padding_mode)[:4]
        return (0 if (src_img is self._pinned or self._pinned is None) else 1, hp, wp, top, left)

    def flow_low(self, copy=True):
        plan = getattr(self, "_low_plan", None)
        if plan is None:
            raise RuntimeError("flow_low(): no flow has been computed yet")
        return plan.flow_low() if copy else plan.flow4.t[:, :2].t().reshape(2, plan.hf, plan.wf)

    def compute_flow(self, src_img, dst_img, mode="TC", vis=False, src_img_identifier=None,
                     numpy_out=False, do_sigmoid=False, borrow=False, defer_weights=False, weight_region=False,
                     src_is_previous_dst=False, visibility=False, flow_init=None, iters=None, flow_region=False):
        if visibility and not self.masked:
            raise ValueError("compute_flow(visibility=True) needs raft_type 'weighted_masked': no other type has a mask output")
        assert mode in ["flow", "TC"]
        assert src_img.shape == dst_img.shape
        if src_img_identifier is not None and self.masked:
            if not self._cache_mask_warned:
                self._cache_mask_warned = True
                logger.warning("raft_type 'weighted_masked': the flow cache holds no visibility mask -- cached flows are not used, "
                               "every flow is computed")
        elif src_img_identifier is not None:
            try:
                return self._cached_flow(src_img, src_img_identifier, mode, numpy_out, do_sigmoid, borrow)
            except Exception as ex:
                key = (type(ex), str(ex))
                if key not in self._cache_errors:
                    self._cache_errors.add(key)
                    logger.warning(f"no cached flow: {ex}")
        H, W = src_img.shape[:2]
        hp, wp, top, left, oh, ow, lh, lw = _pad_geometry(H, W, self.C.padding_mode)
        pinned_here = src_img is self._pinned
        slot = 0 if (pinned_here or self._pinned is None) else 1
        plan = self.engine.plan(hp, wp, slot)
        if flow_init is not None:
            flow_init = self._as_flow_init(flow_init, hp, wp)
        n_iters = int(self.C.iters) if iters is None else int(iters)
        if n_iters < 1:
            raise ValueError("iters must be >= 1")
        self._touch_plan((hp, wp) if slot == 0 else (hp, wp, slot), (oh, ow), plan.P, pinned_here)
        start_time = timer()

        def up(a):
            if isinstance(a, torch.Tensor):
                t = a if a.is_cuda else a.cuda(non_blocking=True)
            else:
                t = torch.from_numpy(np.ascontiguousarray(a)).cuda(non_blocking=True)
            if t.dtype != torch.uint8 or t.dim() != 3 or t.shape[2] != 3:
                raise TypeError(f"compute_flow takes (H, W, 3) uint8 BGR images, got {tuple(t.shape)} {t.dtype}")
            if (lh, lw) != (H, W):
                t = t[:lh, :lw].contiguous()
            return t.contiguous()

        key = (hp, wp, top, left)
        if pinned_here and self._pinned_key == key and plan.source_tag is self:
            pass
        else:
            s = up(src_img)
            plan.load_image(0, s, top, left)
            reuse = bool(src_is_previous_dst) and self._last_dst.get(id(plan)) == (id(src_img), key)
            self.source_features_reused = bool(plan.encode_source(reuse_target=reuse))
            plan.source_tag = self if pinned_here else None
            if pinned_here:
                self._pinned_key = key
        post = self.C.weights_postprocessing_fn or None
        region = None
        if weight_region and not post:
            if pinned_here:
                region = self._weight_region(key, hp, wp, top, left, oh, ow)
            if region is None and defer_weights:
                if plan.P not in self._all_pixels:
                    self._all_pixels[plan.P] = torch.arange(plan.P, dtype=torch.int32, device="cuda")
                region = self._all_pixels[plan.P]
        plan.set_weight_region(region)
        frect = None
        if flow_region and self.flow_region_on and pinned_here and not post and flow_init is None and not self.masked:
            frect = self._flow_region(key, hp, wp, top, left, oh, ow)
        plan.set_flow_region(frect, n_iters)
        d = up(dst_img)
        plan.load_image(1, d, top, left)
        self._last_dst[id(plan)] = (id(dst_img), key)
        o = self._outputs(oh, ow)
        weighted = self.C.raft_type in ("weighted", "weighted_masked")
        self.weights_deferred = bool(defer_weights and weighted and not self.masked and not self.engine.small
                                     and plan.wh_region is not None
                                     and mode == "TC" and not numpy_out
                                     and int(plan.wh_region[0].numel()) > self.defer_min_ratio * int(defer_weights))
        self._deferred = (plan, (top, left), oh, ow, o, bool(do_sigmoid)) if self.weights_deferred else None
        if flow_init is not None:
            plan.set_flow_init(flow_init)
        self._run_flow(plan, n_iters, (top, left), oh, ow, o, weighted, bool(do_sigmoid) and not post,
                       defer_wh=self.weights_deferred, want_flow=(mode == "flow"), mask_sigmoid=bool(visibility),
                       has_init=flow_init is not None)
        self._low_plan, self.last_flow_key = plan, (slot,) + key
        if self.weights_deferred:
            return self._deliver(o, None, mode, oh, ow, numpy_out, borrow)
        logger.debug(f"flow enqueue time [s]: {float(timer() - start_time)}")
        weights = o["w"] if weighted else None
        if post and weights is not None:
            self._postprocess_logits(o, oh, ow, do_sigmoid)
        return self._deliver(o, weights, mode, oh, ow, numpy_out, borrow)
```

### woft_amd/ops.py

```python
import ctypes as C
import math
import os
from dataclasses import dataclass

import numpy as np
import torch

from . import _lib
from ._lib import ConvParams, LookupOtfParams, LookupParams, check, ptr, stream_ptr

DEV = "cuda"


def _round_up(x, m):
    return (x + m - 1) // m * m


@dataclass
class Act:
    t: torch.Tensor
    n: int
    h: int
    w: int
    c: int
# ... 498 lines not shown
    p.wgt_hi, p.wgt_lo, p.precision = ptr(f2_hi), ptr(f2_lo), PRECISION.get(precision, precision)
    p.cout, p.cout_pad = n_q, f2_rows.shape[0]
    p.out, p.ldo, p.co_off = ptr(out), out.shape[1], 0
    p.out_w, p.out_pitch = 0, 0
    p.epi = _lib.EPI_LINEAR
    p.tile_m, p.tile_n = (128, 128) if f2_rows.shape[0] % 128 == 0 else (128, 64)
    p._keep = (f1, f2_rows, out, f2_hi, f2_lo)
    return p


def tiled_dims(h, w, tw=4):
    ht, wt = (h + 3) // 4, (w + tw - 1) // tw
    return ht, wt, ht * wt * 4 * tw


def tile_rows(x, out):
    check(_lib.load().woft_tile_rows(ptr(x.t), x.h, x.w, x.cs, ptr(out), stream_ptr()), "woft_tile_rows")


def tile_planes(planes, tw=4):
    P, h, w = planes.shape
    ht, wt, n = tiled_dims(h, w, tw)
    pad = torch.zeros(P, ht * 4, wt * tw, dtype=planes.dtype, device=planes.device)
    pad[:, :h, :w] = planes
    return pad.reshape(P, ht, 4, wt, tw).permute(0, 1, 3, 2, 4).reshape(P, n).contiguous()


def untile_planes(vol, h, w, tw=4):
    ht, wt, n = tiled_dims(h, w, tw)
    P = vol.shape[0]
    return vol[:, :n].reshape(P, ht, wt, 4, tw).permute(0, 1, 3, 2, 4).reshape(P, ht * 4, wt * tw)[:, :h, :w]


def make_lookup_params(vols, dims, coords, out, radius):
    p = LookupParams()
    assert len({v.dtype for v in vols}) == 1 and vols[0].dtype in (torch.float32, torch.bfloat16)
    p.vol_bf16 = int(vols[0].dtype == torch.bfloat16)
    for l, v in enumerate(vols):
        p.vol[l] = ptr(v)
        p.ht[l], p.wt[l], n = tiled_dims(*dims[l])
        assert v.shape[1] >= n
        p.plane[l] = v.shape[1]
    p.levels, p.radius = len(vols), radius
    p.coords, p.n_pix, p.out, p.ldo = ptr(coords), coords.shape[0], ptr(out), out.shape[1]
    p._keep = (vols, coords, out)
    return p


def run_lookup(p):
    check(_lib.load().woft_corr_lookup(C.byref(p), stream_ptr()), "woft_corr_lookup")


def coords_init(coords, hf, wf, flow4=None, flow_cat=None, ld_cat=0):
    check(_lib.load().woft_coords_init(ptr(coords), hf, wf, ptr(flow4), ptr(flow_cat), ld_cat, stream_ptr()),
          "woft_coords_init")


def coords_init_flow(coords, flow_init, hf, wf, flow4=None, flow_cat=None, ld_cat=0):
    assert flow_init.dtype == torch.float32 and flow_init.is_contiguous() and tuple(flow_init.shape) == (2, hf, wf)
    check(_lib.load().woft_coords_init_flow(ptr(coords), ptr(flow_init), hf, wf, ptr(flow4), ptr(flow_cat), ld_cat,
                                            stream_ptr()), "woft_coords_init_flow")


def forward_interpolate(flow, out=None):
    assert flow.dtype == torch.float32 and flow.is_contiguous() and flow.dim() == 3 and flow.shape[0] == 2
    if out is None:
        out = torch.empty_like(flow)
    assert out.dtype == torch.float32 and out.is_contiguous() and out.shape == flow.shape
    check(_lib.load().woft_forward_interpolate(ptr(flow), flow.shape[1], flow.shape[2], ptr(out), stream_ptr()),
          "woft_forward_interpolate")
    return out


def coords_update(coords, delta, ld_delta, wf, flow4=None, flow_cat=None, ld_cat=0):
    check(_lib.load().woft_coords_update(ptr(coords), ptr(delta), ld_delta, wf, coords.shape[0], ptr(flow4),
                                         ptr(flow_cat), ld_cat, stream_ptr()), "woft_coords_update")


def wh_needed(pts, count, n_max, top, left, hf, wf, index, bitmap, dyn_index, n_needed=None):
    check(_lib.load().woft_wh_needed(ptr(pts), ptr(count), n_max, top, left, hf, wf, ptr(index), index.numel(), ptr(bitmap),
                                     ptr(dyn_index), ptr(n_needed), stream_ptr()), "woft_wh_needed")


def warp_features(f, coords, out):
    check(_lib.load().woft_warp_features(ptr(f.t), f.h, f.w, f.c, f.cs, ptr(coords), out.n_pix, ptr(out.t), out.cs,
                                         stream_ptr()), "woft_warp_features")


def convex_upsample(coords, wlow, mask, hf, wf, crop, h, w, flow_up=None, dst=None, wout=None, do_sigmoid=False):
    check(_lib.load().woft_convex_upsample(ptr(coords), ptr(wlow), ptr(mask), mask.shape[1], hf, wf, crop[0], crop[1],
                                           h, w, ptr(flow_up), ptr(dst), ptr(wout), int(do_sigmoid), stream_ptr()),
          "woft_convex_upsample")


def convex_weights_at(pts, count, n_max, wlow, mask, hf, wf, crop, wsel, do_sigmoid=False):
    check(_lib.load().woft_convex_weights_at(ptr(pts), ptr(count), n_max, ptr(wlow), ptr(mask), mask.shape[1], hf, wf,
                                             crop[0], crop[1], int(do_sigmoid), ptr(wsel), stream_ptr()),
          "woft_convex_weights_at")


def upflow8(coords, wlow, hf, wf, crop, h, w, flow_up=None, dst=None, wout=None, do_sigmoid=False):
    check(_lib.load().woft_upflow8(ptr(coords), ptr(wlow), hf, wf, crop[0], crop[1], h, w, ptr(flow_up), ptr(dst),
                                   ptr(wout), int(do_sigmoid), stream_ptr()), "woft_upflow8")


def warp_perspective_u8(img, Hmat, out=None, valid=None, nearest=False):
    h, w = img.shape[:2]
    c = 1 if img.dim() == 2 else img.shape[2]
    arr = (C.c_double * 9)(*np.linalg.inv(np.asarray(Hmat, dtype=np.float64)).ravel().tolist())
    check(_lib.load().woft_warp_perspective_u8(ptr(img), h, w, c, arr, ptr(out), ptr(valid), int(nearest),
                                               stream_ptr()), "woft_warp_perspective_u8")


def _hinv9(Hmat):
    return (C.c_double * 9)(*np.linalg.inv(np.asarray(Hmat, dtype=np.float64)).ravel().tolist())


def warp_perspective_window_u8(img, Hmat, rect, out=None, valid=None, nearest=False):
    h, w = img.shape[:2]
    c = 1 if img.dim() == 2 else img.shape[2]
    y0, x0, rows, cols = (int(v) for v in rect)
    assert out is None or out.numel() == rows * cols * c
    assert valid is None or valid.numel() == rows * cols
    check(_lib.load().woft_warp_perspective_window_u8(ptr(img), h, w, c, _hinv9(Hmat), y0, x0, rows, cols, ptr(out), ptr(valid),
                                                      int(nearest), stream_ptr()), "woft_warp_perspective_window_u8")


def crop_u8(img, rect, out=None):
    h, w = img.shape[:2]
    c = 1 if img.dim() == 2 else img.shape[2]
    y0, x0, rows, cols = (int(v) for v in rect)
    if out is None:
        out = torch.empty((rows, cols) + tuple(img.shape[2:]), dtype=torch.uint8, device=img.device)
    assert out.numel() == rows * cols * c and out.is_contiguous() and img.is_contiguous()
    check(_lib.load().woft_crop_u8(ptr(img), h, w, c, y0, x0, rows, cols, ptr(out), stream_ptr()), "woft_crop_u8")
    return out


_BBOX_WS = {}


def mask_bbox_ws(device=None):
    dev = torch.device(device or DEV)
    key = (dev.type, dev.index if dev.index is not None else torch.cuda.current_device(), stream_ptr())
    if key not in _BBOX_WS:
        _BBOX_WS[key] = torch.zeros(int(_lib.load().woft_mask_bbox_ws_bytes()), dtype=torch.uint8, device=dev)
    return _BBOX_WS[key]


def mask_bbox(mask, bbox=None, Hmat=None, warped=None, ws=None):
    h, w = mask.shape
    if bbox is None:
        bbox = torch.empty(5, dtype=torch.int32, device=mask.device)
    assert mask.is_contiguous() and (warped is None or (warped.is_contiguous() and warped.numel() == h * w))
    ws = ws if ws is not None else mask_bbox_ws(mask.device)
    check(_lib.load().woft_mask_bbox(ptr(mask), h, w, None if Hmat is None else _hinv9(Hmat), ptr(warped), ptr(ws), ptr(bbox),
                                     stream_ptr()), "woft_mask_bbox")
    return bbox


def resize_by_factor_u8(img, factor):
    h, w = img.shape[:2]
    c = 1 if img.dim() == 2 else img.shape[2]
    ho, wo = int(round(h / factor)), int(round(w / factor))
    out = torch.empty((ho, wo) if img.dim() == 2 else (ho, wo, c), dtype=torch.uint8, device=img.device)
    check(_lib.load().woft_resize_linear_u8(ptr(img), h, w, c, ptr(out), ho, wo, float(factor), float(factor),
                                            stream_ptr()), "woft_resize_linear_u8")
    return out


def tc_select_ws(n):
    return torch.empty(int(_lib.load().woft_tc_select_ws_bytes(n)), dtype=torch.uint8, device=DEV)


def tc_select(dst, w, tmask_u8, pwmask_u8, h, wimg, check_dst, sobol_u, ws, pa, pb, wout, count, grid=None):
    n_draw = 0 if sobol_u is None else sobol_u.numel()
    gh, gw = grid or (h, wimg)
    assert dst.numel() == 2 * gh * gw and tmask_u8.numel() == h * wimg and (w is None or w.numel() == gh * gw)
    check(_lib.load().woft_tc_select(ptr(dst), ptr(w), ptr(tmask_u8), ptr(pwmask_u8), gh, gw, h, wimg, int(check_dst),
                                     ptr(sobol_u), n_draw, ptr(ws), ptr(pa), ptr(pb), ptr(wout), pa.shape[0],
                                     ptr(count), stream_ptr()), "woft_tc_select")


def tc_flags(dst, tmask_u8, pwmask_u8, h, wimg, check_dst, grid=None, out=None):
    gh, gw = grid or (h, wimg)
    assert tmask_u8.numel() == h * wimg and (dst is None or dst.numel() == 2 * gh * gw)
    flags = out if out is not None else torch.empty(gh * gw, dtype=torch.uint8, device=tmask_u8.device)
    check(_lib.load().woft_tc_flags(ptr(dst), ptr(tmask_u8), ptr(pwmask_u8), gh, gw, h, wimg, int(check_dst),
                                    ptr(flags), stream_ptr()), "woft_tc_flags")
    return flags.view(torch.bool)


VIS_MODES = {"gate": 1, "weight": 2}


def tc_select_vis(dst, w, tmask_u8, pwmask_u8, h, wimg, check_dst, sobol_u, vis, vis_mode, vis_thr, ws, pa, pb, wout, count,
                  grid=None):
    n_draw = 0 if sobol_u is None else sobol_u.numel()
    gh, gw = grid or (h, wimg)
    assert dst.numel() == 2 * gh * gw and tmask_u8.numel() == h * wimg and (w is None or w.numel() == gh * gw)
    assert vis is None or (vis.numel() == gh * gw and vis.dtype == torch.float32)
    mode = VIS_MODES[vis_mode] if isinstance(vis_mode, str) else int(vis_mode or 0)
    check(_lib.load().woft_tc_select_vis(ptr(dst), ptr(w), ptr(tmask_u8), ptr(pwmask_u8), gh, gw, h, wimg, int(check_dst),
                                         ptr(sobol_u), n_draw, ptr(vis), mode, float(vis_thr), ptr(ws), ptr(pa), ptr(pb),
                                         ptr(wout), pa.shape[0], ptr(count), stream_ptr()), "woft_tc_select_vis")


def tc_flags_vis(dst, tmask_u8, pwmask_u8, h, wimg, check_dst, vis, vis_mode, vis_thr, grid=None, out=None):
    gh, gw = grid or (h, wimg)
    assert tmask_u8.numel() == h * wimg and (dst is None or dst.numel() == 2 * gh * gw)
    assert vis is None or (vis.numel() == gh * gw and vis.dtype == torch.float32)
    mode = VIS_MODES[vis_mode] if isinstance(vis_mode, str) else int(vis_mode or 0)
    flags = out if out is not None else torch.empty(gh * gw, dtype=torch.uint8, device=tmask_u8.device)
    check(_lib.load().woft_tc_flags_vis(ptr(dst), ptr(tmask_u8), ptr(pwmask_u8), gh, gw, h, wimg, int(check_dst), ptr(vis),
                                        mode, float(vis_thr), ptr(flags), stream_ptr()), "woft_tc_flags_vis")
    return flags.view(torch.bool)


_HFIT_WS = {}


def hfit_ws(device=None):
    dev = torch.device(device or DEV)
    key = (dev.type, dev.index if dev.index is not None else torch.cuda.current_device(), stream_ptr())
    if key not in _HFIT_WS:
        _HFIT_WS[key] = torch.empty(int(_lib.load().woft_hfit_ws_bytes()), dtype=torch.uint8, device=dev)
    return _HFIT_WS[key]


HFIT_SINGLE_MAX = 2048


def hfit(pa, pb, w, Hout, status, count=None, reweight=0, huber_k=1.0, n_irls=0, ws=None):
    n = pa.shape[0]
    if ws is None and n > HFIT_SINGLE_MAX:
        ws = hfit_ws(pa.device)
    check(_lib.load().woft_hfit(ptr(pa), ptr(pb), ptr(w), n, ptr(count), reweight, float(huber_k), n_irls,
                                ptr(ws), ptr(Hout), ptr(status), stream_ptr()), "woft_hfit")


HFIT_BATCH_MAX = 65535


def hfit_batched(pa, pb, w, Hout, status, counts=None, reweight=0, huber_k=1.0, n_irls=0):
    B, n = pa.shape[0], pa.shape[1]
    fn = _lib.load().woft_hfit_batched
    for lo in range(0, B, HFIT_BATCH_MAX):
        hi = min(B, lo + HFIT_BATCH_MAX)
        check(fn(ptr(pa[lo:hi]), ptr(pb[lo:hi]), ptr(w[lo:hi]) if w is not None else None, hi - lo, n,
                 ptr(counts[lo:hi]) if counts is not None else None, reweight, float(huber_k), n_irls, ptr(Hout[lo:hi]),
                 ptr(status[lo:hi]), stream_ptr()), "woft_hfit_batched")


def hfit_batched_bwd(pa, pb, w, gH, gpa, gpb, gw, status=None, counts=None):
    B, n = pa.shape[0], pa.shape[1]
    fn = _lib.load().woft_hfit_batched_bwd
    sl = lambda t, lo, hi: ptr(t[lo:hi]) if t is not None else None
    for lo in range(0, B, HFIT_BATCH_MAX):
        hi = min(B, lo + HFIT_BATCH_MAX)
        check(fn(ptr(pa[lo:hi]), ptr(pb[lo:hi]), sl(w, lo, hi), hi - lo, n, sl(counts, lo, hi), ptr(gH[lo:hi]), sl(gpa, lo, hi),
                 sl(gpb, lo, hi), sl(gw, lo, hi), sl(status, lo, hi), stream_ptr()), "woft_hfit_batched_bwd")


def hfit_step(pa, pb, w, rew, first, res, Hout, status, ws=None):
    ws = ws if ws is not None else hfit_ws(pa.device)
    check(_lib.load().woft_hfit_step(ptr(pa), ptr(pb), ptr(w), pa.shape[0], ptr(rew), int(bool(first)), ptr(ws),
                                     ptr(res), ptr(Hout), ptr(status), stream_ptr()), "woft_hfit_step")


_RANSAC_WS = {}


def ransac_ws(n_max, max_iters, device=None):
    dev = torch.device(device or DEV)
    key = (dev.type, dev.index if dev.index is not None else torch.cuda.current_device(), stream_ptr())
    need = int(_lib.load().woft_ransac_ws_bytes(int(n_max), int(max_iters)))
    if need < 0:
        raise _lib.WoftHipError(f"woft_ransac_ws_bytes({n_max}, {max_iters}) rejected its arguments")
    if key not in _RANSAC_WS or _RANSAC_WS[key].numel() < need:
        _RANSAC_WS[key] = torch.empty(need, dtype=torch.uint8, device=dev)
    return _RANSAC_WS[key]


def ransac(pa, pb, Hout, status, count=None, max_iters=10000, thr=1.4142, conf=0.995, seed=0, refine=True, info=None,
           inlier_mask=None, ws=None):
    n = pa.shape[0]
    ws = ws if ws is not None else ransac_ws(n, max_iters, pa.device)
    check(_lib.load().woft_ransac(ptr(pa), ptr(pb), n, ptr(count), int(max_iters), float(thr), float(conf),
                                  int(seed) & 0xFFFFFFFFFFFFFFFF, int(bool(refine)), ptr(ws), ptr(Hout), ptr(status), ptr(info),
                                  ptr(inlier_mask), stream_ptr()), "woft_ransac")


_TRS_WS = {}


def trs_ws(n_max, max_iters, device=None):
    dev = torch.device(device or DEV)
    key = (dev.type, dev.index if dev.index is not None else torch.cuda.current_device(), stream_ptr())
    need = int(_lib.load().woft_trs_ws_bytes(int(n_max), int(max_iters)))
    if need < 0:
        raise _lib.WoftHipError(f"woft_trs_ws_bytes({n_max}, {max_iters}) rejected its arguments")
    if key not in _TRS_WS or _TRS_WS[key].numel() < need:
        _TRS_WS[key] = torch.empty(need, dtype=torch.uint8, device=dev)
    return _TRS_WS[key]


def trs(pa, pb, Hout, status, count=None, max_iters=10000, thr=3.0, conf=0.999, seed=0, refine=True, info=None,
        inlier_mask=None, ws=None):
    n = pa.shape[0]
    ws = ws if ws is not None else trs_ws(n, max_iters, pa.device)
    check(_lib.load().woft_trs(ptr(pa), ptr(pb), n, ptr(count), int(max_iters), float(thr), float(conf),
                               int(seed) & 0xFFFFFFFFFFFFFFFF, int(bool(refine)), ptr(ws), ptr(Hout), ptr(status), ptr(info),
                               ptr(inlier_mask), stream_ptr()), "woft_trs")


def inlier_frac(pa, pb, Hm, frac, thr=5.0, count=None):
    check(_lib.load().woft_inlier_frac(ptr(pa), ptr(pb), pa.shape[0], ptr(count), ptr(Hm), float(thr), ptr(frac),
                                       stream_ptr()), "woft_inlier_frac")
```

### woft_amd/tracker.py

```python
import logging
import os
import time
from inspect import signature
from types import SimpleNamespace

import numpy as np
import torch

from . import ops
from .homography import compose_H

logger = logging.getLogger(__name__)
_EYE = np.eye(3)


def _count_components(mask_bool):
    from scipy import ndimage
    _, n = ndimage.label(mask_bool, structure=np.ones((3, 3), dtype=bool))
    return n


def make_forward_compatible(subsampler_fn):
    if len(signature(subsampler_fn).parameters) != 3:
        return subsampler_fn
# ... 29 lines not shown
    def __init__(self):
        self.key, self.stage, self.dev, self.done, self.i = None, None, None, None, 0

    def __call__(self, a):
        a = np.asarray(a)
        if a.dtype != np.uint8:
            raise TypeError(f"frames and masks must be uint8, got {a.dtype}")
        key = a.shape
        if key != self.key:
            self.dev = [torch.empty(key, dtype=torch.uint8, device="cuda") for _ in range(2)]
            if self.STAGED:
                self.stage = [torch.empty(key, dtype=torch.uint8).pin_memory() for _ in range(2)]
                self.done = [torch.cuda.Event(), torch.cuda.Event()]
            self.key, self.i = key, 0
        i = self.i = self.i ^ 1
        if not self.STAGED:
            self.dev[i].copy_(torch.from_numpy(np.ascontiguousarray(a)))
            return self.dev[i]
        self.done[i].synchronize()
        if a.flags.c_contiguous and a.nbytes >= (1 << 20):
            from . import _lib
            _lib.check(_lib.load().woft_upload_u8(a.ctypes.data, self.stage[i].data_ptr(), self.dev[i].data_ptr(), a.nbytes, 4,
                                                  _lib.stream_ptr()), "woft_upload_u8")
        else:
            np.copyto(self.stage[i].numpy(), a)
            self.dev[i].copy_(self.stage[i], non_blocking=True)
        self.done[i].record()
        return self.dev[i]


class _Fit(SimpleNamespace):
    """Result of one solve: H (3x3 float64, cur -> src) and, for the global stage, the re-detection verdict."""


class YAOFTrackerSingleControl:
    DEVICE = "cuda"

    VISIBILITY_MODES = ("gate", "weight")

    def _visibility_config(self):
        C = self.C
        mode = C.visibility_mode
        if isinstance(mode, type(C)) or not mode:
            return None, 0.5
        if mode not in self.VISIBILITY_MODES:
            raise ValueError(f"visibility_mode {mode!r}: not one of {self.VISIBILITY_MODES} (or absent / None: the mask is not used)")
        if C.flow_config.raft_type != "weighted_masked":
            raise ValueError(f"visibility_mode {mode!r} needs a flow config with raft_type 'weighted_masked' (the MaskHead computes the "
                             f"visibility); this one has {C.flow_config.raft_type!r}")
        thr = C.visibility_thr
        thr = 0.5 if (isinstance(thr, type(C)) or thr is None) else thr
        try:
            thr = float(thr)
        except (TypeError, ValueError):
            raise ValueError(f"visibility_thr {thr!r}: not a float in (0, 1)") from None
        if not 0.0 < thr < 1.0:
            raise ValueError(f"visibility_thr {thr!r}: not a float in (0, 1)")
        return mode, float(np.float32(thr))

    def _warm_start_config(self):
        C = self.C
        on = C.warm_start_local
        on = False if isinstance(on, type(C)) else bool(on)
        n = C.warm_start_iters
        if isinstance(n, type(C)) or n is None:
            return on, None
        if isinstance(n, bool) or not isinstance(n, (int, np.integer)) or n < 1:
            raise ValueError(f"warm_start_iters {n!r}: not an integer >= 1")
        return on, int(n)

    def __init__(self, config):
        self.C = config
        self.warm_start_local, self.warm_start_iters = self._warm_start_config()
        self.local_warm_started = False
        self._warm = None
        self.visibility_mode, self.visibility_thr = self._visibility_config()
        if config.flow_config.raft_type == "weighted_masked" and self.visibility_mode is None:
            raise ValueError("the tracker takes a flow config with raft_type 'orig' or 'weighted'; 'weighted_masked' (MaskHead "
                             "visibility mask) returns a mask the tracker does not consume unless visibility_mode = 'gate' or "
                             "'weight' is set")
        if self.C.subsampler_fn:
            self.C.subsampler_fn = make_forward_compatible(self.C.subsampler_fn)
        self.flower = config.flow_config.of_class(config.flow_config)
        self.device = self.DEVICE
        self._fused = self._fused_specs()
        self._sparse_weights = False
        self.n_kept = None
        self._replay = None
        self._announced = False
        self._local_chain = None
        self._n_tracked = 0
        self._upload = _FrameUploader()
        self.host_wait_s = 0.0

    def _fused_specs(self):
        self.solver_decision = None
        spec = self._fused_specs_plain()
        if self.visibility_mode is not None:
            self.solver_decision += (f"; visibility {self.visibility_mode}"
                                     + (f" (p > {self.visibility_thr:.9g})" if self.visibility_mode == "gate" else " (w * p)"))
        return spec

    def _fused_specs_plain(self):
        C = self.C
        self.solver_decision = "callable back end"
        v = C.device_solver
        if os.environ.get("WOFT_FUSED", "1") == "0" or (not isinstance(v, type(C)) and v is not None and not v):
            self.solver_decision += " (device back end switched off)"
            return None
        if C.post_hoc_weights_postprocessing_fn or C.flow_numpy_out:
            return None
        if not hasattr(self.flower, "pin_source"):
            return None
        if self.flower.C.raft_type != ("weighted" if self.visibility_mode is None else "weighted_masked"):
            return None
        from .probe import solver_spec
        spec, how = solver_spec(C.H_estimator, C.subsampler_fn or None, C.redet_success_fn, device=self.device)
        self.solver_decision = ("device back end" if spec is not None else "callable back end") + f" ({how})"
        probed = spec is not None and "probed" in how
        logger.log(logging.WARNING if probed else logging.INFO,
                   f"tracker solver: {self.solver_decision}"
                   + (" -- the config's estimator / subsampler / re-detection callables were recognised by behavioural probing and "
                      "are replaced by the HIP solver (same results, tested); set `device_solver = False` in the tracker config "
                      "(or WOFT_FUSED=0) to run the config's own callables instead" if probed else ""))
        if spec is None:
            return None
        from .presets import sobol_points
        n_draw = spec["n_draw"]
        spec["sobol_u"] = torch.from_numpy(sobol_points(n_draw).astype(np.float32)).to(self.device) if n_draw else None
        return spec

    def _fused_buffers(self, n_grid):
        if getattr(self, "_fb_key", None) != n_grid:
            cap = 1024 if self._fused["n_draw"] else n_grid
            self._fb = dict(ws=ops.tc_select_ws(n_grid), pa=torch.empty(cap, 2, device=self.device),
                            pb=torch.empty(cap, 2, device=self.device), w=torch.empty(cap, device=self.device),
                            res=torch.zeros(16, dtype=torch.float32, device=self.device),
                            fit_ws=ops.hfit_ws(self.device) if cap > ops.HFIT_SINGLE_MAX else None)
            R = self._fused.get("ransac")
            if R is not None:
                self._fb["fit_ws"] = ops.ransac_ws(cap, R["max_iters"], self.device)
            T = self._fused.get("trs")
            if T is not None:
                self._fb["fit_ws"] = ops.trs_ws(cap, T["max_iters"], self.device)
            self._fb_key = n_grid
        return self._fb

    def init(self, img, mask, img_identifier=None):
        k = self.C.downscale_inputs
        if k:
            img = ops.resize_by_factor_u8(_device_u8(img), k)
            mask = ops.resize_by_factor_u8(_device_u8(mask), k)
            img_identifier = None
        mask_np = mask.cpu().numpy() if isinstance(mask, torch.Tensor) else np.asarray(mask)
        inside = mask_np > 0
        assert _count_components(inside) == 1
        self.template_img = img
        self.np_template_mask = mask_np
        self._local_chain = None
        self._warm = None
        self.template_mask = torch.from_numpy(inside).to(self.device)
        self._template_mask_u8 = torch.from_numpy(inside.astype(np.uint8) * 255).to(self.device)
        if hasattr(self.flower, "pin_source"):
            self.flower.pin_source(self.template_img)
            if hasattr(self.flower, "pin_weight_region"):
                self.flower.pin_weight_region(inside if self._mask_weight_head() else None)
# ... 9 lines not shown
        self._replay = None

    def set_fast_meta(self, meta):
        if self.C.downscale_inputs:
            raise NotImplementedError("Fastforward not compatible with input downscaling yet.")
        self._replay = meta

    @property
    def fast_forward(self):
        return self._replay is not None

    @fast_forward.setter
    def fast_forward(self, value):
        if not value:
            self._replay = None
        elif self._replay is None:
            raise ValueError("fast_forward = True needs set_fast_meta(meta)")

    def track(self, input_img, debug=False, img_identifier=None):
        if self.C.downscale_inputs:
            input_img = ops.resize_by_factor_u8(_device_u8(input_img), self.C.downscale_inputs)
        if self._replay is not None:
            meta, self._replay = self._replay, None
            self._warm = None
            H_cur2init = meta.estim_H_current2template
            self.lost, self.N_lost = False, 0
            self.prev_H2init = self.last_good_H2init = H_cur2init
            self.prev_img = input_img.clone() if isinstance(input_img, torch.Tensor) else np.array(input_img)
            self.prev_img_identifier = img_identifier
            return H_cur2init, meta

        meta = SimpleNamespace()
        self._n_tracked += 1
        if self.C.no_prewarp_after_N and self.N_lost > self.C.no_prewarp_after_N:
            self.last_good_H2init = _EYE.copy()
        meta.last_good_H2init = self.last_good_H2init.copy()
        frame = _device_u8(input_img, copy=True) if isinstance(input_img, torch.Tensor) else self._upload(input_img)

        prewarp_H = self.last_good_H2init
        fit = self._global_stage(frame, prewarp_H)
        if self.visibility_mode is not None:
            meta.n_kept = self.n_kept
        H_global = compose_H(prewarp_H, fit.H)
        meta.H_global_cur2init = H_global.copy()
        logger.debug(f"global_H_success: {fit.success}")
        if fit.success:
            self.lost, self.N_lost = False, 0
            self._warm = None
            H_cur2init = H_global
        else:
            self.lost, self.N_lost = True, self.N_lost + 1
            H_cur2init = H_global
            if not self.C.no_local_H:
                H_cur2init = meta.H_local_cur2init = self._local_stage(frame)
                meta.local_warm_started = self.local_warm_started
                if self.visibility_mode is not None:
                    meta.n_kept_local = self.n_kept
        if debug:
            logger.debug("debug visualisation (TRK:210-264) needs the OpenCV GUI and is not part of the HIP path")

        self.prev_img, self.prev_img_identifier = frame, img_identifier
        self._set_pose(H_cur2init.copy(), good=not self.lost)
        meta.lost, meta.N_lost, meta.global_H_success = self.lost, self.N_lost, fit.success
        if not self._announced:
            self._announced = True
            meta.precision = getattr(self.flower, "precision", None)
            meta.precision_source = getattr(self.flower, "precision_source", None)
            meta.solver_decision = self.solver_decision
            if self.visibility_mode is not None:
                meta.visibility_mode = self.visibility_mode
        k = self.C.downscale_inputs
        if k:
            H_cur2init = compose_H(np.diag([1.0 / k, 1.0 / k, 1.0]), H_cur2init, np.diag([float(k), float(k), 1.0]))
        return H_cur2init, meta

    def _mask_weight_head(self):
        if self.C.post_hoc_weights_postprocessing_fn:
            return False
        v = self.C.mask_weight_head
        if isinstance(v, type(self.C)) or v is None:
            return os.environ.get("WOFT_MASK_WEIGHT_HEAD", "1") != "0"
        return bool(v)

    def _flow_region_on(self):
        return bool(self._mask_weight_head() and self.visibility_mode is None and not self.warm_start_local)

    def _set_pose(self, H, good):
        self.prev_H2init = H
        if good:
            self.last_good_H2init = H.copy()

    def _flow(self, src, dst, src_is_previous_dst=False, flow_init=None, iters=None, flow_region=False):
        kw = {"borrow": True, "weight_region": True} if hasattr(self.flower, "pin_source") else {}
        if self._sparse_weights:
            kw["defer_weights"] = int(self._fused["n_draw"])
        if src_is_previous_dst and "borrow" in kw:
            kw["src_is_previous_dst"] = True
        if flow_region and hasattr(self.flower, "pin_flow_region"):
            kw["flow_region"] = True
        if flow_init is not None:
            kw["flow_init"] = flow_init
            if iters is not None:
                kw["iters"] = iters
        self.n_kept = None
        p = None
        if self.visibility_mode is not None:
            src_xy, dst_xy, w, p = self.flower.compute_flow(src, dst, mode="TC", vis=False, src_img_identifier=None,
                                                            do_sigmoid=True, visibility=True, **kw)
        else:
            src_xy, dst_xy, w = self.flower.compute_flow(src, dst, mode="TC", vis=False, src_img_identifier=None,
                                                         do_sigmoid=True, **kw)
        s = getattr(self.flower, "last_flow_shape", None)
        return src_xy, dst_xy, w, p, ((s["H"], s["W"]) if s else None)

    def _global_stage(self, frame, prewarp_H):
        valid = None
        if np.array_equal(prewarp_H, _EYE):
            prewarped = frame
        else:
            key = tuple(frame.shape)
            if getattr(self, "_pw_key", None) != key:
                self._pw_buf = (torch.empty_like(frame), torch.empty(frame.shape[:2], dtype=torch.uint8, device=self.device))
                self._pw_key = key
            prewarped, valid = self._pw_buf
            ops.warp_perspective_u8(frame, prewarp_H, prewarped, valid)
        if self.C.do_not_mask_TCs_by_prewarped:
            valid = None
        src_xy, dst_xy, w, p, grid = self._flow(self.template_img, prewarped, flow_region=self._flow_region_on())
        return self._solve(src_xy, dst_xy, w, grid, frame.shape[:2], self._template_mask_u8, valid, bounds=True,
                           judge=True, vis=p)

    def _local_stage(self, frame):
        chained = (self._local_chain is not None and self._local_chain[0] is self.prev_img and self._local_chain[1] == self._n_tracked - 1
                   and os.environ.get("WOFT_LOCAL_REUSE", "1") != "0")
        init, self.local_warm_started = None, False
        if self.warm_start_local:
            ran = (self._local_chain is not None and self._local_chain[0] is self.prev_img
                   and self._local_chain[1] == self._n_tracked - 1)
            if ran and self._warm is not None and self._warm[1] == self.flower.flow_key(self.prev_img):
                from .warm import forward_interpolate
                init = forward_interpolate(self._warm[0])
            self.local_warm_started = init is not None
        src_xy, dst_xy, w, p, grid = self._flow(self.prev_img, frame, src_is_previous_dst=chained, flow_init=init,
                                                iters=self.warm_start_iters)
        self._local_chain = (frame, self._n_tracked)
        if self.warm_start_local:
            self._warm = (self.flower.flow_low(), self.flower.last_flow_key)
        if np.array_equal(self.prev_H2init, _EYE):
            prev_mask = self._template_mask_u8
        else:
            prev_mask = torch.empty_like(self._template_mask_u8)
            ops.warp_perspective_u8(self._template_mask_u8, np.linalg.inv(self.prev_H2init), prev_mask, None,
                                    nearest=True)
        try:
            fit = self._solve(src_xy, dst_xy, w, grid, frame.shape[:2], prev_mask, None, bounds=False, judge=False, vis=p)
            if not np.all(np.isfinite(fit.H)):
                raise FloatingPointError("singular homography system")
            return compose_H(fit.H, self.prev_H2init)
        except Exception as ex:
            logger.warning(f"frame-to-frame homography failed ({type(ex).__name__}): pose of the previous frame kept")
            return self.prev_H2init

    def _solve(self, src_xy, dst_xy, w, grid, frame_hw, src_mask_u8, dst_valid_u8, bounds, judge, vis=None):
        Hh, Ww = frame_hw
        grid = grid or (Hh, Ww)
        try:
            if self._fused is not None:
                return self._solve_device(dst_xy, w, grid, (Hh, Ww), src_mask_u8, dst_valid_u8, bounds, vis)
            return self._solve_callables(src_xy, dst_xy, w, grid, (Hh, Ww), src_mask_u8, dst_valid_u8, bounds, judge, vis)
        except AssertionError:
            if self.visibility_mode is None or not judge or self.n_kept is None or self.n_kept >= 4:
                raise
            logger.debug(f"global stage: {self.n_kept} correspondences after the visibility {self.visibility_mode}: no fit")
            return _Fit(H=_EYE.copy(), success=False)

    def _solve_device(self, dst_xy, w, grid, frame_hw, src_mask_u8, dst_valid_u8, bounds, vis=None):
        F, b = self._fused, self._fused_buffers(grid[0] * grid[1])
        res = b["res"]
        ires = res.view(torch.int32)
        weighted = F.get("weighted", True)
        if vis is not None:
            ops.tc_select_vis(dst_xy, w if weighted else None, src_mask_u8, dst_valid_u8, frame_hw[0], frame_hw[1], bounds,
                              F["sobol_u"], vis, self.visibility_mode, self.visibility_thr, b["ws"], b["pa"], b["pb"], b["w"],
                              ires[12:14], grid=grid)
            weighted = weighted or self.visibility_mode == "weight"
        elif w is None and getattr(self.flower, "weights_deferred", False):
            ops.tc_select(dst_xy, None, src_mask_u8, dst_valid_u8, frame_hw[0], frame_hw[1], bounds, F["sobol_u"], b["ws"],
                          b["pa"], b["pb"], b["w"], ires[12:14], grid=grid)
            if weighted:
                self.flower.finish_weights(b["pb"], ires[12:13], b["pb"].shape[0], out=b["w"])
        else:
            ops.tc_select(dst_xy, w, src_mask_u8, dst_valid_u8, frame_hw[0], frame_hw[1], bounds, F["sobol_u"], b["ws"],
                          b["pa"], b["pb"], b["w"], ires[12:14], grid=grid)
        R, T = F.get("ransac"), F.get("trs")
        if R is not None:
            ops.ransac(b["pa"], b["pb"], res[0:9], ires[10:11], count=ires[12:13], max_iters=R["max_iters"], thr=R["thr"],
                       conf=R["conf"], ws=b["fit_ws"])
        elif T is not None:
            ops.trs(b["pa"], b["pb"], res[0:9], ires[10:11], count=ires[12:13], max_iters=T["max_iters"], thr=T["thr"],
                    conf=T["conf"], ws=b["fit_ws"])
        else:
            ops.hfit(b["pa"], b["pb"], b["w"] if weighted else None, res[0:9], ires[10:11], count=ires[12:13],
                     reweight=F["reweight"], huber_k=F["huber_k"], n_irls=F["n_irls"], ws=b["fit_ws"])
        ops.inlier_frac(b["pa"], b["pb"], res[0:9], res[9:10], thr=F["thr"], count=ires[12:13])
        if getattr(self, "_host_res", None) is None:
            self._host_res = torch.empty(16, dtype=torch.float32).pin_memory()
            self._host_ev = torch.cuda.Event()
        host = self._host_res
        host.copy_(res, non_blocking=True)
        self._host_ev.record()
        t0 = time.perf_counter()
        self._host_ev.synchronize()
        self.host_wait_s += time.perf_counter() - t0
        ih = host.view(torch.int32)
        self.n_kept = int(ih[13])
        if int(ih[10]) == 1:
            raise AssertionError(torch.Size([1, int(ih[12]), 2]))
        verdict = F.get("const_verdict")
        if verdict is None:
            verdict = bool(np.float32(host[9]) > np.float32(F["min_frac"]))
        return _Fit(H=host[0:9].numpy().astype(np.float64).reshape(3, 3), success=bool(verdict))

    def _solve_callables(self, src_xy, dst_xy, w, grid, frame_hw, src_mask_u8, dst_valid_u8, bounds, judge, vis=None):
        C = self.C
        post = None
        if C.post_hoc_weights_postprocessing_fn:
            post = self.flower.postprocess_weights(w.clone(), C.post_hoc_weights_postprocessing_fn)
        if vis is None:
            keep = ops.tc_flags(dst_xy if bounds else None, src_mask_u8, dst_valid_u8, frame_hw[0], frame_hw[1], bounds,
                                grid=grid)
        else:
            keep = ops.tc_flags_vis(dst_xy if bounds else None, src_mask_u8, dst_valid_u8, frame_hw[0], frame_hw[1], bounds,
                                    vis, self.visibility_mode, self.visibility_thr, grid=grid)
        pick = lambda t: None if t is None else t[:, keep]
        src_xy, dst_xy, w, post = pick(src_xy), pick(dst_xy), pick(w), pick(post)
        if vis is not None:
            self.n_kept = int(src_xy.shape[1])
            if self.n_kept == 0:
                raise AssertionError(torch.Size([1, 0, 2]))
            if self.visibility_mode == "weight":
                pk = vis.reshape(1, -1)[:, keep]
                w = pk if w is None else w * pk
        if judge:
            src_xy = src_xy.float()
        if C.flow_numpy_out and not judge:
            to_np = lambda t: None if t is None else t.cpu().numpy()
            src_xy, dst_xy, w, post = to_np(src_xy), to_np(dst_xy), to_np(w), to_np(post)
        if C.subsampler_fn:
            src_xy, dst_xy, w, post = C.subsampler_fn(src_xy, dst_xy, w, post)
        if not judge:
            src_xy = src_xy.float() if isinstance(src_xy, torch.Tensor) else src_xy.astype(np.float32)
        H = C.H_estimator(dst_xy.T[None], src_xy.T[None], w)
        H = H.float() if isinstance(H, torch.Tensor) else torch.as_tensor(np.asarray(H)).float()
        fit = _Fit(H=H.detach().cpu().numpy()[0].astype(np.float64), success=None)
        if judge:
            fit.success = bool(C.redet_success_fn(H, src_xy, dst_xy, post if post is not None else w))
        return fit


class WOFTWindow(YAOFTrackerSingleControl):
    PLAN_BOUND = 4
    MIN_FLOW_SIDE = 16

    def __init__(self, config):
        v = config.warm_start_local
        if not isinstance(v, type(config)) and v:
            raise NotImplementedError("warm_start_local is not provided by the search-window tracker: its frame t-1 -> t flows run "
                                      "on a window that follows the object, so consecutive flows do not share a grid")
        super().__init__(config)
        from collections import OrderedDict
        self._fb_cache = OrderedDict()
        self.search_bbox = self.local_search_bbox = None
        if hasattr(self.flower, "bound_plans"):
            self.flower.bound_plans(self.PLAN_BOUND)

    def init(self, img, mask, img_identifier=None):
        from . import window
        super().init(img, mask, img_identifier)
        inside = self.np_template_mask > 0
        Hh, Ww = inside.shape
        self._margin = self.C.search_window_margin or None
        self._template_box = window.Box.from_mask(inside)
        self.search_bbox = window.search_box(self._template_box, self._margin, Ww, Hh)
        self.local_search_bbox = None
        self._rect = rect = self.search_bbox.crop_rect()
        y0, x0, rows, cols = rect
        self._template_crop = ops.crop_u8(_device_u8(self.template_img), rect)
# ... 77 lines not shown
```

Measured before the change: 125.4.

## Fuse point weighting, homography fit and inlier fraction into one launch

Adds a single-block kernel that computes per-point convex-upsample weights, runs the IRLS homography fit, and evaluates the inlier fraction in one launch. This replaces the separate weights, hfit and inlier_frac launches. A wh_needed_clear variant also zeroes the low-res weight map inside the needed-window kernel, so the separate zero_ call is dropped. Both paths are enabled by default through a tail_fused flag. The aim is to cut launch count and latency on the serial tail of each frame, at the cost of doing the weight computation inside a single block.

```diff
diff --git a/include/woft_hip.h b/include/woft_hip.h
--- a/include/woft_hip.h
+++ b/include/woft_hip.h
@@ -169,6 +169,10 @@
 int woft_wh_needed(const float* pts, const int32_t* count, int32_t n_max, int32_t top, int32_t left, int32_t hf, int32_t wf,
                    const int32_t* index, int32_t n_win, int32_t* bitmap, int32_t* dyn_index, int32_t* n_needed, void* stream);
 
+int woft_wh_needed_clear(const float* pts, const int32_t* count, int32_t n_max, int32_t top, int32_t left, int32_t hf,
+                         int32_t wf, const int32_t* index, int32_t n_win, int32_t* bitmap, int32_t* dyn_index,
+                         int32_t* n_needed, float* wlow, void* stream);
+
 int woft_convex_upsample(const float* coords1, const float* wlow, const float* mask, int32_t ld_mask,
                          int32_t hf, int32_t wf, int32_t crop_top, int32_t crop_left, int32_t h, int32_t w,
                          float* flow_up, float* dst, float* wout, int32_t do_sigmoid, void* stream);
@@ -214,6 +218,10 @@
 int64_t woft_hfit_ws_bytes(void);
 int woft_hfit(const float* pa, const float* pb, const float* w, int32_t n_max, const int32_t* count,
               int32_t reweight, float huber_k, int32_t n_irls, void* ws, float* Hout, int32_t* status, void* stream);
+int woft_hfit_solve_points(const float* pa, const float* pb, float* w, int32_t use_w, int32_t n_max, const int32_t* count,
+                           const float* wlow, const float* mask, int32_t ld_mask, int32_t hf, int32_t wf, int32_t crop_top,
+                           int32_t crop_left, int32_t do_sigmoid, int32_t reweight, float huber_k, int32_t n_irls, float thr,
+                           float* Hout, int32_t* status, float* frac, void* stream);
 #define WOFT_HFIT_BATCH_MAX 65535
 int woft_hfit_batched(const float* pa, const float* pb, const float* w, int32_t batch, int32_t n_max,
                       const int32_t* counts, int32_t reweight, float huber_k, int32_t n_irls, float* Hout,
diff --git a/woft_amd/_lib.py b/woft_amd/_lib.py
--- a/woft_amd/_lib.py
+++ b/woft_amd/_lib.py
@@ -83,6 +83,7 @@
     "woft_wh_reduce": (i32, [vp, i32, i32, vp, f32, i64, vp, vp]),
     "woft_warp_features": (i32, [vp, i32, i32, i32, i32, vp, i64, vp, i32, vp]),
     "woft_wh_needed": (i32, [vp, vp, i32, i32, i32, i32, i32, vp, i32, vp, vp, vp, vp]),
+    "woft_wh_needed_clear": (i32, [vp, vp, i32, i32, i32, i32, i32, vp, i32, vp, vp, vp, vp, vp]),
     "woft_convex_upsample": (i32, [vp, vp, vp, i32, i32, i32, i32, i32, i32, i32, vp, vp, vp, i32, vp]),
     "woft_convex_weights_at": (i32, [vp, vp, i32, vp, vp, i32, i32, i32, i32, i32, i32, vp, vp]),
     "woft_upflow8": (i32, [vp, vp, i32, i32, i32, i32, i32, i32, vp, vp, vp, i32, vp]),
@@ -99,6 +100,8 @@
     "woft_tc_flags_vis": (i32, [vp, vp, vp, i32, i32, i32, i32, i32, vp, i32, f32, vp, vp]),
     "woft_hfit_ws_bytes": (i64, []),
     "woft_hfit": (i32, [vp, vp, vp, i32, vp, i32, f32, i32, vp, vp, vp, vp]),
+    "woft_hfit_solve_points": (i32, [vp, vp, vp, i32, i32, vp, vp, vp, i32, i32, i32, i32, i32, i32, i32, f32, i32, f32, vp, vp,
+                                     vp, vp]),
     "woft_hfit_batched": (i32, [vp, vp, vp, i32, i32, vp, i32, f32, i32, vp, vp, vp]),
     "woft_hfit_batched_bwd": (i32, [vp, vp, vp, i32, i32, vp, vp, vp, vp, vp, vp, vp]),
     "woft_hfit_step": (i32, [vp, vp, vp, i32, vp, i32, vp, vp, vp, vp, vp]),
diff --git a/woft_amd/csrc/hfit.hip b/woft_amd/csrc/hfit.hip
--- a/woft_amd/csrc/hfit.hip
+++ b/woft_amd/csrc/hfit.hip
@@ -1,4 +1,5 @@
 #include "common.h"
+#include "point_weight.h"
 #include <algorithm>
 
 namespace {
@@ -48,8 +49,45 @@
     return 1.f / (a + 1e-8f);
 }
 
+__device__ __forceinline__ bool chol8_factor(const double* gram, double (&L)[36]) {
+    bool ok = true;
+#pragma unroll
+    for (int i = 0; i < 8; ++i) {
+#pragma unroll
+        for (int j = 0; j <= i; ++j) {
+            double s = gram[i * 9 + j];
+#pragma unroll
+            for (int k = 0; k < j; ++k) s -= L[i * (i + 1) / 2 + k] * L[j * (j + 1) / 2 + k];
+            if (i == j) {
+                ok = ok && (s > 0.0);
+                L[i * (i + 1) / 2 + i] = sqrt(s);
+            } else {
+                L[i * (i + 1) / 2 + j] = s / L[j * (j + 1) / 2 + j];
+            }
+        }
+    }
+    return ok;
+}
+
+__device__ __forceinline__ void chol8_solve_f64(const double (&L)[36], double (&rhs)[8]) {
+#pragma unroll
+    for (int i = 0; i < 8; ++i) {
+        double s = rhs[i];
+#pragma unroll
+        for (int k = 0; k < i; ++k) s -= L[i * (i + 1) / 2 + k] * rhs[k];
+        rhs[i] = s / L[i * (i + 1) / 2 + i];
+    }
+#pragma unroll
+    for (int i = 7; i >= 0; --i) {
+        double s = rhs[i];
+#pragma unroll
+        for (int k = i + 1; k < 8; ++k) s -= L[k * (k + 1) / 2 + i] * rhs[k];
+        rhs[i] = s / L[i * (i + 1) / 2 + i];
+    }
+}
+
 __device__ __forceinline__ void hfit_one(const float* __restrict__ pa, const float* __restrict__ pb,
-                                         const float* __restrict__ w, int n, int reweight, float huber_k, int n_solves,
+                                         const float* w, int n, int reweight, float huber_k, int n_solves,
                                          float* __restrict__ Hout, int* __restrict__ status) {
     __shared__ double red[(HT / 64) * 81];
     __shared__ double tot[NG];
@@ -137,34 +175,12 @@
         }
         __syncthreads();
         if (threadIdx.x == 0) {
-            double L[8][8], rhs[8];
-            double G[9][9];
-            for (int a = 0; a < 9; ++a)
-                for (int b = 0; b < 9; ++b) G[a][b] = gram[a * 9 + b];
-            bool ok = true;
-            for (int i = 0; i < 8 && ok; ++i) {
-                for (int j = 0; j <= i; ++j) {
-                    double s = G[i][j];
-                    for (int k = 0; k < j; ++k) s -= L[i][k] * L[j][k];
-                    if (i == j) {
-                        if (!(s > 0.0)) { ok = false; break; }
-                        L[i][i] = sqrt(s);
-                    } else {
-                        L[i][j] = s / L[j][j];
-                    }
-                }
-            }
-            if (ok) {
-                for (int i = 0; i < 8; ++i) {
-                    double s = G[i][8];
-                    for (int k = 0; k < i; ++k) s -= L[i][k] * rhs[k];
-                    rhs[i] = s / L[i][i];
-                }
-                for (int i = 7; i >= 0; --i) {
-                    double s = rhs[i];
-                    for (int k = i + 1; k < 8; ++k) s -= L[k][i] * rhs[k];
-                    rhs[i] = s / L[i][i];
-                }
+            double L[36], rhs[8];
+            if (chol8_factor(gram, L)) {
+#pragma unroll
+                for (int i = 0; i < 8; ++i) rhs[i] = gram[i * 9 + 8];
+                chol8_solve_f64(L, rhs);
+#pragma unroll
                 for (int i = 0; i < 8; ++i) sol_s[i] = (float)rhs[i];
             } else {
                 fail_s = 1;
@@ -185,19 +201,26 @@
         const double i2 = 1.0 / (double)s2;
         const double T2i[9] = {i2, 0, -(double)t2x * i2, 0, i2, -(double)t2y * i2, 0, 0, 1};
         double tmp[9], hh[9];
+#pragma unroll
         for (int r = 0; r < 3; ++r)
+#pragma unroll
             for (int c = 0; c < 3; ++c) {
                 double s = 0;
+#pragma unroll
                 for (int k = 0; k < 3; ++k) s += hn[r * 3 + k] * T1[k * 3 + c];
                 tmp[r * 3 + c] = s;
             }
+#pragma unroll
         for (int r = 0; r < 3; ++r)
+#pragma unroll
             for (int c = 0; c < 3; ++c) {
                 double s = 0;
+#pragma unroll
                 for (int k = 0; k < 3; ++k) s += T2i[r * 3 + k] * tmp[k * 3 + c];
                 hh[r * 3 + c] = s;
             }
         const double den = hh[8] + 1e-8;
+#pragma unroll
         for (int i = 0; i < 9; ++i) Hout[i] = (float)(hh[i] / den);
         status[0] = 0;
     }
@@ -225,43 +248,6 @@
              status + b);
 }
 
-
-__device__ __forceinline__ bool chol8_factor(const double* gram, double (&L)[36]) {
-    bool ok = true;
-#pragma unroll
-    for (int i = 0; i < 8; ++i) {
-#pragma unroll
-        for (int j = 0; j <= i; ++j) {
-            double s = gram[i * 9 + j];
-#pragma unroll
-            for (int k = 0; k < j; ++k) s -= L[i * (i + 1) / 2 + k] * L[j * (j + 1) / 2 + k];
-            if (i == j) {
-                ok = ok && (s > 0.0);
-                L[i * (i + 1) / 2 + i] = sqrt(s);
-            } else {
-                L[i * (i + 1) / 2 + j] = s / L[j * (j + 1) / 2 + j];
-            }
-        }
-    }
-    return ok;
-}
-
-__device__ __forceinline__ void chol8_solve_f64(const double (&L)[36], double (&rhs)[8]) {
-#pragma unroll
-    for (int i = 0; i < 8; ++i) {
-        double s = rhs[i];
-#pragma unroll
-        for (int k = 0; k < i; ++k) s -= L[i * (i + 1) / 2 + k] * rhs[k];
-        rhs[i] = s / L[i * (i + 1) / 2 + i];
-    }
-#pragma unroll
-    for (int i = 7; i >= 0; --i) {
-        double s = rhs[i];
-#pragma unroll
-        for (int k = i + 1; k < 8; ++k) s -= L[k * (k + 1) / 2 + i] * rhs[k];
-        rhs[i] = s / L[i * (i + 1) / 2 + i];
-    }
-}
 
 __device__ __forceinline__ void bwd_zero_rows(float* __restrict__ gpa, float* __restrict__ gpb, float* __restrict__ gw, int from,
                                               int n_max) {
@@ -526,15 +512,12 @@
                  (gw != nullptr) ? gw + off : nullptr, (status != nullptr) ? status + b : nullptr);
 }
 
-__global__ __launch_bounds__(HT) void inlier_frac_kernel(const float* __restrict__ pa, const float* __restrict__ pb,
-                                                         int n_max, const int* __restrict__ count,
-                                                         const float* __restrict__ H, float thr,
-                                                         float* __restrict__ frac) {
+__device__ __forceinline__ void inlier_frac_one(const float* __restrict__ pa, const float* __restrict__ pb, int n,
+                                                const float* H, float thr, float* frac) {
     __shared__ double red[HT / 64];
     __shared__ double tot[1];
-    int n = n_max;
-    if (count != nullptr) n = min(count[0], n_max);
     float h[9];
+#pragma unroll
     for (int i = 0; i < 9; ++i) h[i] = H[i];
     double c[1] = {0.0};
     for (int i = threadIdx.x; i < n; i += HT) {
@@ -546,6 +529,42 @@
     }
     block_sum<1>(c, red, tot);
     if (threadIdx.x == 0) frac[0] = (n > 0) ? (float)(tot[0] / n) : 0.f;
+}
+
+__global__ __launch_bounds__(HT) void inlier_frac_kernel(const float* __restrict__ pa, const float* __restrict__ pb,
+                                                         int n_max, const int* __restrict__ count,
+                                                         const float* __restrict__ H, float thr,
+                                                         float* __restrict__ frac) {
+    int n = n_max;
+    if (count != nullptr) n = min(count[0], n_max);
+    inlier_frac_one(pa, pb, n, H, thr, frac);
+}
+
+struct PointWeights {
+    const float* wlow;
+    const float* mask;
+    int ld_mask, hf, wf, crop_top, crop_left, do_sigmoid;
+};
+
+__global__ __launch_bounds__(HT) void hfit_solve_points_kernel(const float* __restrict__ pa, const float* __restrict__ pb,
+                                                               float* w, int use_w, int n_max,
+                                                               const int* __restrict__ count, PointWeights pw, int reweight,
+                                                               float huber_k, int n_solves, float thr, float* Hout,
+                                                               int* status, float* frac) {
+    int n = n_max;
+    if (count != nullptr) n = min(count[0], n_max);
+    if (pw.wlow != nullptr) {
+        for (int i = threadIdx.x; i < n; i += HT) {
+            const int X = (int)pb[2 * i] + pw.crop_left, Y = (int)pb[2 * i + 1] + pw.crop_top;
+            w[i] = convex_weight_at_pixel(X, Y, pw.wlow, pw.mask, pw.ld_mask, pw.hf, pw.wf, pw.do_sigmoid);
+        }
+        __threadfence_block();
+        __syncthreads();
+    }
+    hfit_one(pa, pb, use_w ? w : nullptr, n, reweight, huber_k, n_solves, Hout, status);
+    __threadfence_block();
+    __syncthreads();
+    inlier_frac_one(pa, pb, n, Hout, thr, frac);
 }
 
 constexpr int MT = 256;
@@ -889,6 +908,21 @@
     return woft_launch_status();
 }
 
+extern "C" int woft_hfit_solve_points(const float* pa, const float* pb, float* w, int32_t use_w, int32_t n_max,
+                                      const int32_t* count, const float* wlow, const float* mask, int32_t ld_mask, int32_t hf,
+                                      int32_t wf, int32_t crop_top, int32_t crop_left, int32_t do_sigmoid, int32_t reweight,
+                                      float huber_k, int32_t n_irls, float thr, float* Hout, int32_t* status, float* frac,
+                                      void* stream) {
+    if (!pa || !pb || !Hout || !status || !frac || n_max < 1 || n_max > WOFT_HFIT_SINGLE_MAX || reweight < 0 || reweight > 2 ||
+        n_irls < 0 || (use_w && !w))
+        return WOFT_EINVAL;
+    if (wlow != nullptr && (!w || !mask || hf <= 0 || wf <= 0 || ld_mask < 576)) return WOFT_EINVAL;
+    const PointWeights pw = {wlow, mask, ld_mask, hf, wf, crop_top, crop_left, do_sigmoid};
+    hipLaunchKernelGGL(hfit_solve_points_kernel, dim3(1), dim3(HT), 0, (hipStream_t)stream, pa, pb, w, use_w, n_max, count, pw,
+                       reweight, huber_k, n_irls + 1, thr, Hout, status, frac);
+    return woft_launch_status();
+}
+
 extern "C" int woft_hfit_batched(const float* pa, const float* pb, const float* w, int32_t batch, int32_t n_max,
                                  const int32_t* counts, int32_t reweight, float huber_k, int32_t n_irls, float* Hout,
                                  int32_t* status, void* stream) {
diff --git a/woft_amd/csrc/point_weight.h b/woft_amd/csrc/point_weight.h
--- /dev/null
+++ b/woft_amd/csrc/point_weight.h
@@ -0,0 +1,34 @@
+#pragma once
+#include "common.h"
+
+__device__ __forceinline__ float convex_weight_at_pixel(int X, int Y, const float* __restrict__ wlow,
+                                                        const float* __restrict__ mask, int ld_mask, int hf, int wf,
+                                                        int do_sigmoid) {
+    const int hc = Y >> 3, wc = X >> 3, lane = (Y & 7) * 8 + (X & 7);
+    const float* m = mask + ((int64_t)hc * wf + wc) * ld_mask + lane;
+    float e[9];
+    float mx = -INFINITY;
+#pragma unroll
+    for (int k = 0; k < 9; ++k) {
+        e[k] = m[k * 64];
+        mx = fmaxf(mx, e[k]);
+    }
+    float den = 0.f;
+#pragma unroll
+    for (int k = 0; k < 9; ++k) {
+        e[k] = expf(e[k] - mx);
+        den += e[k];
+    }
+    float aw = 0.f;
+#pragma unroll
+    for (int k = 0; k < 9; ++k) {
+        const int ny = hc + k / 3 - 1, nx = wc + k % 3 - 1;
+        float vw = 0.f;
+        if (ny >= 0 && ny < hf && nx >= 0 && nx < wf) vw = 8.f * wlow[(int64_t)ny * wf + nx];
+        const float s = e[k] / den;
+        aw += s * vw;
+    }
+    float v = aw / 8.f;
+    if (do_sigmoid) v = sigmoidf_(v);
+    return v;
+}
diff --git a/woft_amd/csrc/upsample.hip b/woft_amd/csrc/upsample.hip
--- a/woft_amd/csrc/upsample.hip
+++ b/woft_amd/csrc/upsample.hip
@@ -1,4 +1,5 @@
 #include "common.h"
+#include "point_weight.h"
 #include "warp_pixel.h"
 
 namespace {
@@ -66,33 +67,7 @@
     const int n = count ? min(count[0], n_max) : n_max;
     if (i >= n) return;
     const int X = (int)pts[2 * i] + crop_left, Y = (int)pts[2 * i + 1] + crop_top;
-    const int hc = Y >> 3, wc = X >> 3, lane = (Y & 7) * 8 + (X & 7);
-    const float* m = mask + ((int64_t)hc * wf + wc) * ld_mask + lane;
-    float e[9];
-    float mx = -INFINITY;
-#pragma unroll
-    for (int k = 0; k < 9; ++k) {
-        e[k] = m[k * 64];
-        mx = fmaxf(mx, e[k]);
-    }
-    float den = 0.f;
-#pragma unroll
-    for (int k = 0; k < 9; ++k) {
-        e[k] = expf(e[k] - mx);
-        den += e[k];
-    }
-    float aw = 0.f;
-#pragma unroll
-    for (int k = 0; k < 9; ++k) {
-        const int ny = hc + k / 3 - 1, nx = wc + k % 3 - 1;
-        float vw = 0.f;
-        if (ny >= 0 && ny < hf && nx >= 0 && nx < wf) vw = 8.f * wlow[(int64_t)ny * wf + nx];
-        const float s = e[k] / den;
-        aw += s * vw;
-    }
-    float v = aw / 8.f;
-    if (do_sigmoid) v = sigmoidf_(v);
-    wsel[i] = v;
+    wsel[i] = convex_weight_at_pixel(X, Y, wlow, mask, ld_mask, hf, wf, do_sigmoid);
 }
 
 __global__ void upflow8_kernel(const float* __restrict__ coords1, const float* __restrict__ wlow, int hf, int wf,
diff --git a/woft_amd/csrc/wh.hip b/woft_amd/csrc/wh.hip
--- a/woft_amd/csrc/wh.hip
+++ b/woft_amd/csrc/wh.hip
@@ -155,6 +155,56 @@
     if (need && n_needed != nullptr) atomicAdd(n_needed, 1);
 }
 
+constexpr int WH_ONE_T = 1024;
+constexpr int WH_ONE_MAX_CELLS = 262144;
+__global__ __launch_bounds__(WH_ONE_T) void wh_needed_one_kernel(const float* __restrict__ pts, const int* __restrict__ count,
+                                                                  int n_max, int top, int left, int hf, int wf,
+                                                                  const int* __restrict__ index, int n_win,
+                                                                  int* __restrict__ bitmap, int* __restrict__ dyn,
+                                                                  int* __restrict__ n_needed, float* __restrict__ wlow) {
+    __shared__ unsigned bits[WH_ONE_MAX_CELLS / 32];
+    __shared__ int wsum[WH_ONE_T / 64];
+    const int P = hf * wf, words = (P + 31) >> 5;
+    for (int k = threadIdx.x; k < words; k += WH_ONE_T) bits[k] = 0u;
+    __syncthreads();
+    const int n = count ? min(count[0], n_max) : n_max;
+    for (int i = threadIdx.x; i < n; i += WH_ONE_T) {
+        const int cx = ((int)pts[2 * i] + left) >> 3, cy = ((int)pts[2 * i + 1] + top) >> 3;
+#pragma unroll
+        for (int dy = -1; dy <= 1; ++dy)
+#pragma unroll
+            for (int dx = -1; dx <= 1; ++dx) {
+                const int yy = cy + dy, xx = cx + dx;
+                if (yy >= 0 && yy < hf && xx >= 0 && xx < wf) {
+                    const int c = yy * wf + xx;
+                    atomicOr(&bits[c >> 5], 1u << (c & 31));
+                }
+            }
+    }
+    __syncthreads();
+    for (int c = threadIdx.x; c < P; c += WH_ONE_T) {
+        bitmap[c] = (int)((bits[c >> 5] >> (c & 31)) & 1u);
+        if (wlow != nullptr) wlow[c] = 0.f;
+    }
+    int cnt = 0;
+    for (int j = threadIdx.x; j < n_win; j += WH_ONE_T) {
+        const int src = index[j];
+        const bool need = src >= 0 && src < P && ((bits[src >> 5] >> (src & 31)) & 1u) != 0u;
+        dyn[j] = need ? src : -1;
+        cnt += need ? 1 : 0;
+    }
+    if (n_needed == nullptr) return;
+#pragma unroll
+    for (int o = 32; o > 0; o >>= 1) cnt += __shfl_xor(cnt, o);
+    if ((threadIdx.x & 63) == 0) wsum[threadIdx.x >> 6] = cnt;
+    __syncthreads();
+    if (threadIdx.x == 0) {
+        int t = 0;
+        for (int k = 0; k < WH_ONE_T / 64; ++k) t += wsum[k];
+        n_needed[0] = t;
+    }
+}
+
 extern "C" int woft_wh_needed(const float* pts, const int32_t* count, int32_t n_max, int32_t top, int32_t left, int32_t hf,
                               int32_t wf, const int32_t* index, int32_t n_win, int32_t* bitmap, int32_t* dyn_index,
                               int32_t* n_needed, void* stream) {
@@ -169,6 +219,21 @@
     return woft_launch_status();
 }
 
+extern "C" int woft_wh_needed_clear(const float* pts, const int32_t* count, int32_t n_max, int32_t top, int32_t left,
+                                    int32_t hf, int32_t wf, const int32_t* index, int32_t n_win, int32_t* bitmap,
+                                    int32_t* dyn_index, int32_t* n_needed, float* wlow, void* stream) {
+    if (!pts || !index || !bitmap || !dyn_index || n_max <= 0 || n_win <= 0 || hf <= 0 || wf <= 0) return WOFT_EINVAL;
+    if ((int64_t)hf * wf > WH_ONE_MAX_CELLS) {
+        const int rc = woft_wh_needed(pts, count, n_max, top, left, hf, wf, index, n_win, bitmap, dyn_index, n_needed, stream);
+        if (rc != WOFT_OK) return rc;
+        if (wlow) (void)hipMemsetAsync(wlow, 0, (size_t)hf * wf * sizeof(float), (hipStream_t)stream);
+        return woft_launch_status();
+    }
+    hipLaunchKernelGGL(wh_needed_one_kernel, dim3(1), dim3(WH_ONE_T), 0, (hipStream_t)stream, pts, count, n_max, top, left, hf,
+                       wf, index, n_win, bitmap, dyn_index, n_needed, wlow);
+    return woft_launch_status();
+}
+
 extern "C" int woft_wh_conv0(const float* lookup, int32_t ld_lookup, const float* mean, int64_t n_pix, int32_t nwin,
                              const float* wt, const float* bias, float* out, const int32_t* index, void* stream) {
     if (!lookup || !mean || !wt || !bias || !out || n_pix <= 0 || n_pix >= (1ll << 31)) return WOFT_EINVAL;
diff --git a/woft_amd/engine.py b/woft_amd/engine.py
--- a/woft_amd/engine.py
+++ b/woft_amd/engine.py
@@ -289,6 +289,8 @@
         self._fold = self._fold_gather_programs()
         self.flow_region = None
         self._flow_regions = {}
+        self.tail_fused = os.environ.get("WOFT_TAIL_FUSED", "1") != "0"
+        self.wh_sums_valid = False
         if eng.weighted:
             n = sp.nwin
             self.x8 = new_act(P, n, n, 5, cs=8, zero=True)
@@ -703,6 +705,7 @@
 
     def encode_source(self, reuse_target=False):
         reused = bool(reuse_target) and self.otf and getattr(self, "target_valid", False)
+        self.wh_sums_valid = False
         if reused:
             self.f1rows[:self.P].copy_(self.f2act[0].t.view(self.P, -1))
             if self.prec != "fp32":
@@ -734,6 +737,10 @@
         self.run(self.prog_f_dst)
         self.run(self.prog_volume)
         self.target_valid = True
+        self.wh_sums_valid = False
+        if e.weighted and self.tail_fused and getattr(self, "wh0_direct", False):
+            self._wh_target_sums()
+            self.wh_sums_valid = True
         off = sp.flow_off
         if flow_init is None:
             ops.coords_init(self.coords, self.hf, self.wf, self.flow4.t, self.xbuf.t[:, off:], self.xbuf.cs)
@@ -807,8 +814,13 @@
             self._wh_dyn[key] = (dyn, prog, torch.zeros(self.P, dtype=torch.int32, device=index.device),
                                  torch.zeros(1, dtype=torch.int32, device=index.device))
         dyn, prog, bitmap, n_needed = self._wh_dyn[key]
-        ops.wh_needed(pts, count, n_max, pad[0], pad[1], self.hf, self.wf, index, bitmap, dyn, n_needed)
-        self._weight_head(prog, dyn, n_needed, need=bitmap)
+        if self.tail_fused:
+            ops.wh_needed_clear(pts, count, n_max, pad[0], pad[1], self.hf, self.wf, index, bitmap, dyn, n_needed, self.wlow)
+        else:
+            ops.wh_needed(pts, count, n_max, pad[0], pad[1], self.hf, self.wf, index, bitmap, dyn, n_needed)
+        self._weight_head(prog, dyn, n_needed, need=bitmap, wlow_cleared=self.tail_fused)
+        if w_points is True:
+            return (self.wlow, self.mask.t, self.hf, self.wf, crop, do_sigmoid)
         if w_points is not None:
             ops.convex_weights_at(pts, count, n_max, self.wlow, self.mask.t, self.hf, self.wf, crop, w_points,
                                   do_sigmoid=do_sigmoid)
@@ -822,7 +834,15 @@
             self._wh6_pad[:self.eng.wh6_c] = self.eng.wh6_w[:self.eng.wh6_c]
         return self._wh6_pad
 
-    def _weight_head(self, prog_wh, index, n_needed=None, need=None):
+    def _wh_target_sums(self):
+        sp, lib = self.eng.spec, _lib.load()
+        _lib.check(lib.woft_colsum(_lib.ptr(self.f2act[0].t), self.P, sp.fdim, _lib.ptr(self.cs_ws), 256,
+                                   _lib.ptr(self.cs_tot), _lib.stream_ptr()), "woft_colsum")
+        _lib.check(lib.woft_wh_pack(_lib.ptr(self.corr.t), self.corr.cs, _lib.ptr(self.f1.t), sp.fdim,
+                                    _lib.ptr(self.cs_tot), 1.0 / (math.sqrt(float(sp.fdim)) * self.P), self.P, sp.nwin,
+                                    _lib.ptr(self.wmean), None, _lib.stream_ptr()), "woft_wh_pack")
+
+    def _weight_head(self, prog_wh, index, n_needed=None, need=None, wlow_cleared=False):
         e, sp = self.eng, self.eng.spec
         if need is not None and self.otf:
             self.lookup.need = _lib.ptr(need)
@@ -832,16 +852,17 @@
             self._lookup(self.lookup)
         lib = _lib.load()
         n = sp.nwin
-        _lib.check(lib.woft_colsum(_lib.ptr(self.f2act[0].t), self.P, sp.fdim, _lib.ptr(self.cs_ws), 256,
-                                   _lib.ptr(self.cs_tot), _lib.stream_ptr()), "woft_colsum")
-        _lib.check(lib.woft_wh_pack(_lib.ptr(self.corr.t), self.corr.cs, _lib.ptr(self.f1.t), sp.fdim,
-                                    _lib.ptr(self.cs_tot), 1.0 / (math.sqrt(float(sp.fdim)) * self.P), self.P, n,
-                                    _lib.ptr(self.wmean), None if self.wh0_direct else _lib.ptr(self.x8.t),
-                                    _lib.stream_ptr()), "woft_wh_pack")
+        if not (self.wh_sums_valid and self.wh0_direct):
+            _lib.check(lib.woft_colsum(_lib.ptr(self.f2act[0].t), self.P, sp.fdim, _lib.ptr(self.cs_ws), 256,
+                                       _lib.ptr(self.cs_tot), _lib.stream_ptr()), "woft_colsum")
+            _lib.check(lib.woft_wh_pack(_lib.ptr(self.corr.t), self.corr.cs, _lib.ptr(self.f1.t), sp.fdim,
+                                        _lib.ptr(self.cs_tot), 1.0 / (math.sqrt(float(sp.fdim)) * self.P), self.P, n,
+                                        _lib.ptr(self.wmean), None if self.wh0_direct else _lib.ptr(self.x8.t),
+                                        _lib.stream_ptr()), "woft_wh_pack")
         if not e.wh_std and not e.wh_flat0:
             self.x32.t[:, :8].copy_(self.x8.t)
         n_win = int(index.numel()) if index is not None else self.P
-        if index is not None:
+        if index is not None and not wlow_cleared:
             self.wlow.zero_()
         if self.wh0_direct and not self.wh0_fused:
             _lib.check(lib.woft_wh_conv0(_lib.ptr(self.corr.t), self.corr.cs, _lib.ptr(self.wmean), n_win, n,
diff --git a/woft_amd/flow_provider.py b/woft_amd/flow_provider.py
--- a/woft_amd/flow_provider.py
+++ b/woft_amd/flow_provider.py
@@ -118,6 +118,8 @@
                                  volume_storage=getattr(self.C, "volume_storage", None), mask_head=self.masked)
         v = getattr(self.C, "flow_region", None)
         self.flow_region_on = (os.environ.get("WOFT_FLOW_REGION", "1") != "0") if (v is None or isinstance(v, type(self.C))) else bool(v)
+        v = getattr(self.C, "tail_fused", None)
+        self.tail_fused_on = (os.environ.get("WOFT_TAIL_FUSED", "1") != "0") if (v is None or isinstance(v, type(self.C))) else bool(v)
         self.use_graph = (os.environ.get("WOFT_GRAPH") or str(int(bool(getattr(self.C, "graph", False))))) == "1"
         self._pinned = None
         self._pinned_key = None
@@ -172,9 +174,11 @@
         else:
             g.replay()
 
-    def finish_weights(self, pts, count, n_max, out=None):
+    def finish_weights(self, pts, count, n_max, out=None, in_solve=False):
         plan, crop, oh, ow, o, do_sigmoid = self._deferred
         self._deferred = None
+        if in_solve:
+            return plan.finish_weights(pts, count, n_max, crop, crop, oh, ow, do_sigmoid=do_sigmoid, w_points=True)
         plan.finish_weights(pts, count, n_max, crop, crop, oh, ow, flow_up=o["flow"], dst=o["dst"], wout=o["w"],
                             do_sigmoid=do_sigmoid, w_points=out)
         return o["w"] if out is None else out
@@ -372,6 +376,7 @@
         if flow_region and self.flow_region_on and pinned_here and not post and flow_init is None and not self.masked:
             frect = self._flow_region(key, hp, wp, top, left, oh, ow)
         plan.set_flow_region(frect, n_iters)
+        plan.tail_fused = self.tail_fused_on
         d = up(dst_img)
         plan.load_image(1, d, top, left)
         self._last_dst[id(plan)] = (id(dst_img), key)
diff --git a/woft_amd/ops.py b/woft_amd/ops.py
--- a/woft_amd/ops.py
+++ b/woft_amd/ops.py
@@ -604,6 +604,12 @@
                                      ptr(dyn_index), ptr(n_needed), stream_ptr()), "woft_wh_needed")
 
 
+def wh_needed_clear(pts, count, n_max, top, left, hf, wf, index, bitmap, dyn_index, n_needed, wlow):
+    check(_lib.load().woft_wh_needed_clear(ptr(pts), ptr(count), n_max, top, left, hf, wf, ptr(index), index.numel(),
+                                           ptr(bitmap), ptr(dyn_index), ptr(n_needed), ptr(wlow), stream_ptr()),
+          "woft_wh_needed_clear")
+
+
 def warp_features(f, coords, out):
     check(_lib.load().woft_warp_features(ptr(f.t), f.h, f.w, f.c, f.cs, ptr(coords), out.n_pix, ptr(out.t), out.cs,
                                          stream_ptr()), "woft_warp_features")
@@ -761,6 +767,15 @@
                                 ptr(ws), ptr(Hout), ptr(status), stream_ptr()), "woft_hfit")
 
 
+def hfit_solve_points(pa, pb, w, Hout, status, frac, count=None, reweight=0, huber_k=1.0, n_irls=0, thr=5.0, use_w=True,
+                      point_weights=None):
+    wlow, mask, hf, wf, crop, do_sigmoid = point_weights if point_weights is not None else (None, None, 0, 0, (0, 0), False)
+    check(_lib.load().woft_hfit_solve_points(ptr(pa), ptr(pb), ptr(w), int(bool(use_w)), pa.shape[0], ptr(count), ptr(wlow),
+                                             ptr(mask), mask.shape[1] if mask is not None else 0, hf, wf, crop[0], crop[1],
+                                             int(do_sigmoid), reweight, float(huber_k), n_irls, float(thr), ptr(Hout),
+                                             ptr(status), ptr(frac), stream_ptr()), "woft_hfit_solve_points")
+
+
 HFIT_BATCH_MAX = 65535
 
 
diff --git a/woft_amd/tracker.py b/woft_amd/tracker.py
--- a/woft_amd/tracker.py
+++ b/woft_amd/tracker.py
@@ -135,6 +135,9 @@
         if self.C.subsampler_fn:
             self.C.subsampler_fn = make_forward_compatible(self.C.subsampler_fn)
         self.flower = config.flow_config.of_class(config.flow_config)
+        v = self.C.tail_fused
+        if not (isinstance(v, type(self.C)) or v is None) and hasattr(self.flower, "tail_fused_on"):
+            self.flower.tail_fused_on = bool(v)
         self.device = self.DEVICE
         self._fused = self._fused_specs()
         self._sparse_weights = False
@@ -310,6 +313,12 @@
             return os.environ.get("WOFT_MASK_WEIGHT_HEAD", "1") != "0"
         return bool(v)
 
+    def _tail_fused(self):
+        v = self.C.tail_fused
+        if isinstance(v, type(self.C)) or v is None:
+            return os.environ.get("WOFT_TAIL_FUSED", "1") != "0"
+        return bool(v)
+
     def _flow_region_on(self):
         return bool(self._mask_weight_head() and self.visibility_mode is None and not self.warm_start_local)
 
@@ -407,6 +416,9 @@
         res = b["res"]
         ires = res.view(torch.int32)
         weighted = F.get("weighted", True)
+        one_launch = (self._tail_fused() and F.get("ransac") is None and F.get("trs") is None
+                      and b["pa"].shape[0] <= ops.HFIT_SINGLE_MAX)
+        point_weights = None
         if vis is not None:
             ops.tc_select_vis(dst_xy, w if weighted else None, src_mask_u8, dst_valid_u8, frame_hw[0], frame_hw[1], bounds,
                               F["sobol_u"], vis, self.visibility_mode, self.visibility_thr, b["ws"], b["pa"], b["pb"], b["w"],
@@ -415,7 +427,9 @@
         elif w is None and getattr(self.flower, "weights_deferred", False):
             ops.tc_select(dst_xy, None, src_mask_u8, dst_valid_u8, frame_hw[0], frame_hw[1], bounds, F["sobol_u"], b["ws"],
                           b["pa"], b["pb"], b["w"], ires[12:14], grid=grid)
-            if weighted:
+            if weighted and one_launch and getattr(self.flower, "tail_fused_on", False):
+                point_weights = self.flower.finish_weights(b["pb"], ires[12:13], b["pb"].shape[0], in_solve=True)
+            elif weighted:
                 self.flower.finish_weights(b["pb"], ires[12:13], b["pb"].shape[0], out=b["w"])
         else:
             ops.tc_select(dst_xy, w, src_mask_u8, dst_valid_u8, frame_hw[0], frame_hw[1], bounds, F["sobol_u"], b["ws"],
@@ -427,10 +441,15 @@
         elif T is not None:
             ops.trs(b["pa"], b["pb"], res[0:9], ires[10:11], count=ires[12:13], max_iters=T["max_iters"], thr=T["thr"],
                     conf=T["conf"], ws=b["fit_ws"])
+        elif one_launch:
+            ops.hfit_solve_points(b["pa"], b["pb"], b["w"], res[0:9], ires[10:11], res[9:10], count=ires[12:13],
+                                  reweight=F["reweight"], huber_k=F["huber_k"], n_irls=F["n_irls"], thr=F["thr"],
+                                  use_w=weighted, point_weights=point_weights)
         else:
             ops.hfit(b["pa"], b["pb"], b["w"] if weighted else None, res[0:9], ires[10:11], count=ires[12:13],
                      reweight=F["reweight"], huber_k=F["huber_k"], n_irls=F["n_irls"], ws=b["fit_ws"])
-        ops.inlier_frac(b["pa"], b["pb"], res[0:9], res[9:10], thr=F["thr"], count=ires[12:13])
+        if not one_launch:
+            ops.inlier_frac(b["pa"], b["pb"], res[0:9], res[9:10], thr=F["thr"], count=ires[12:13])
         if getattr(self, "_host_res", None) is None:
             self._host_res = torch.empty(16, dtype=torch.float32).pin_memory()
             self._host_ev = torch.cuda.Event()
```

Result: no change. 126.0, median of 6 (+0.5%).
